# instance-based-loc/instance-based-loc

Hardware: AMD Instinct MI355X
Metric: query-frames localized/sec (embed+match+register) (higher is better)
Workload: dtype f16 (ViT MFMA operands, f32 accumulate) / f32+f64 (match, registration); 1 GPU; T: dinov2_vitb14 crops 224^2 (Q=7), 10000-instance memory (E=4), FPFH+RANSAC+coloured ICP on 5000-pt clouds, whole-memory evaluate; synthetic objects of extent U[0.15, 0.6] m on a 2.50 m grid (SURVEY 8d's U[0.2, 1.5] m re-scoped: its 5 000 points are too sparse to survive the radius-outlier removal); memory_instances=10000, points_per_object=5000, resident_feature_bytes_per_point=264, parallelism=frames-dp1+memory-replicated

## Files before the change

instance-based-loc_amd/csrc/vit.hip:

```cpp
#include "vit_kernels.h"

__global__ void ibl_set_prefix_kernel(float* __restrict__ x, const float* __restrict__ cls_pos, const float* __restrict__ reg, int B, int T,
                                      int n_prefix, int dim) {
    const int64_t i = (int64_t)blockIdx.x * blockDim.x + threadIdx.x;
    if (i >= (int64_t)B * n_prefix * dim) return;
    const int c = (int)(i % dim);
    const int64_t br = i / dim;
    const int b = (int)(br / n_prefix), r = (int)(br % n_prefix);
    x[((int64_t)b * T + r) * dim + c] = r == 0 ? cls_pos[c] : reg[(int64_t)(r - 1) * dim + c];
}

static int64_t vit_layout(const ibl_vit_desc* d, int batch, int64_t offs[IBL_VIT_WS_COUNT], int64_t* payload = nullptr) {
    const int64_t R = rows_pad((int64_t)batch * d->n_tokens);
    const int at = (d->flags & IBL_VIT_ACT_TERMS3) ? 3 : ((d->flags & IBL_VIT_ACT_TERMS2) ? 2 : 1);
    int64_t bytes[IBL_VIT_WS_COUNT];
    bytes[IBL_VIT_WS_X] = R * d->dim * 4;
    bytes[IBL_VIT_WS_XN] = R * d->dim * 2 * 3;
    bytes[IBL_VIT_WS_QKV] = R * 3 * d->dim * 2;
    bytes[IBL_VIT_WS_ATT] = R * d->dim * 2 * at;
    bytes[IBL_VIT_WS_HID] = R * d->mlp_dim * 2 * at;
    bytes[IBL_VIT_WS_FIN] = rows_pad(batch) * d->dim * 2;
    int64_t p = 0, sum = 0;
    for (int i = 0; i < IBL_VIT_WS_COUNT; ++i) {
        p = (p + 255) & ~(int64_t)255;
        offs[i] = p;
        p += bytes[i];
        sum += bytes[i];
    }
    if (payload) *payload = sum;
    return p;
}

extern "C" int64_t ibl_vit_workspace_bytes(const ibl_vit_desc* d, int batch) {
    if (!d || batch <= 0) return -1;
    int64_t offs[IBL_VIT_WS_COUNT], sum = 0;
    vit_layout(d, batch, offs, &sum);
    return sum + rows_pad(batch) * d->dim * 4 + 9 * 256;
}

extern "C" int ibl_vit_workspace_layout(const ibl_vit_desc* d, int batch, int64_t* offsets, int n) {
    if (!d || batch <= 0 || !offsets || n < 0 || n > IBL_VIT_WS_COUNT)
        return ibl_set_error(IBL_ERR_ARG, "ibl_vit_workspace_layout: bad argument");
    int64_t offs[IBL_VIT_WS_COUNT];
    vit_layout(d, batch, offs);
    for (int i = 0; i < n; ++i) offsets[i] = offs[i];
    return IBL_OK;
}

struct VitCtx {
    const ibl_vit_desc* d;
    const ibl_vit_weights* w;
    int batch;
    hipStream_t s;
    float* x;
    u16 *xn, *qkv, *att, *hid, *fin;
    int64_t Rn;
    int at;
    int n_prefix;
};


static int embed(const VitCtx& c, const void* patches) {
    const ibl_vit_desc* d = c.d;
    const ibl_vit_weights* w = c.w;
    const int D = d->dim, T = d->n_tokens, P = T - c.n_prefix;
    int st;
    GemmEpi e{};
    e.bias = w->b_patch; e.pos = w->pos_patch; e.out = c.x; e.ldo = D; e.tokens_per_crop = T; e.patches_per_crop = P;
    e.patch_row0 = c.n_prefix;
    st = gemm_launch(IBL_LINEAR_PATCH_F32, IBL_ACT_GELU_ERF, reinterpret_cast<const u16*>(patches), d->patch_k_pad,
                     reinterpret_cast<const u16*>(w->w_patch), d->patch_k_pad, c.batch * P, D, d->patch_k_pad, e, c.s);
    if (st) return st;
    if (w->w_patch_lo) {
        GemmEpi e2 = e;
        e2.bias = nullptr; e2.accumulate = 1; e2.alpha = 1.0f / IBL_VIT_SPLIT_SCALE; e2.algo_k = -1;
        st = gemm_launch(IBL_LINEAR_PATCH_F32, IBL_ACT_GELU_ERF, reinterpret_cast<const u16*>(patches), d->patch_k_pad,
                         reinterpret_cast<const u16*>(w->w_patch_lo), d->patch_k_pad, c.batch * P, D, d->patch_k_pad, e2, c.s);
        if (st) return st;
    }
    if (!(d->flags & IBL_VIT_NO_CLS)) {
        const int64_t n = (int64_t)c.batch * c.n_prefix * D;
        hipLaunchKernelGGL(ibl_set_prefix_kernel, dim3((unsigned)((n + 255) / 256)), dim3(256), 0, c.s, c.x, w->cls_pos, w->reg_tokens, c.batch,
                           T, c.n_prefix, D);
        IBL_LAUNCH_CHECK();
    }
    if (d->flags & IBL_VIT_PRE_LN) {
        st = launch_layernorm(c.x, D, c.Rn, D, w->ln_pre_g, w->ln_pre_b, d->ln_eps, c.x, D, 0, c.s);
        if (st) return st;
    }
    return IBL_OK;
}

static int resid_gemm(const VitCtx& c, bool cls_only, const u16* a, int64_t lda, int rows, int terms, int K, const void* w, const void* w_x,
                      const void* w_lo, const float* bias, const float* ls, const float* ls_lo) {
    const int D = c.d->dim;
    GemmEpi e{};
    e.bias = bias; e.scale = ls; e.out = c.x; e.ldo = cls_only ? (int64_t)c.d->n_tokens * D : D; e.alpha = 1.0f; e.algo_k = K;
    const int64_t kx = (int64_t)terms * K;
    int st = gemm_launch((ls || !gemm_resid_pre()) ? IBL_LINEAR_RESID_F32 : IBL_LINEAR_RESID_PRE_F32, IBL_ACT_GELU_ERF, a, lda,
                         reinterpret_cast<const u16*>(terms > 1 ? w_x : w), kx, rows, D, (int)kx, e, c.s);
    if (st) return st;
    if (!cls_only && terms == 1 && w_lo) {
        e.bias = nullptr; e.scale = ls_lo; e.algo_k = -1; e.alpha = 1.0f / IBL_VIT_SPLIT_SCALE;
        st = gemm_launch(ls_lo ? IBL_LINEAR_RESID_F32 : IBL_LINEAR_RESID_PRE_F32, IBL_ACT_GELU_ERF, a, K, reinterpret_cast<const u16*>(w_lo), K, rows,
                         D, K, e, c.s);
    }
    return st;
}

static int attention_half(const VitCtx& c, int l, const BlockTerms& t) {
    const ibl_vit_desc* d = c.d;
    const ibl_vit_layer* L = &c.w->layers[l];
    const int D = d->dim, T = d->n_tokens, H = d->heads;
    const int64_t TD = (int64_t)T * D;
    int st = launch_layernorm(c.x, D, c.Rn, D, L->ln1_g, L->ln1_b, d->ln_eps, c.xn, (int64_t)t.qkv * D, t.qkv, c.s);
    if (st) return st;
    if (!t.cls_only) {
        GemmEpi e{};
        e.bias = L->b_qkv; e.out = c.qkv; e.ldo = 3 * D; e.algo_k = D;
        st = gemm_launch(IBL_LINEAR_F16, IBL_ACT_GELU_ERF, c.xn, (int64_t)t.qkv * D, reinterpret_cast<const u16*>(t.qkv > 1 ? L->w_qkv_x : L->w_qkv),
                         (int64_t)t.qkv * D, (int)c.Rn, 3 * D, t.qkv * D, e, c.s);
        if (st) return st;
    } else {
        GemmEpi e{};
        e.bias = L->b_qkv + D; e.out = c.qkv + D; e.ldo = 3 * D;
        st = gemm_launch(IBL_LINEAR_F16, IBL_ACT_GELU_ERF, c.xn, D, reinterpret_cast<const u16*>(L->w_qkv) + (int64_t)D * D, D, (int)c.Rn, 2 * D, D, e,
                         c.s);
        if (st) return st;
        GemmEpi q{};
        q.bias = L->b_qkv; q.out = c.qkv; q.ldo = 3 * TD;
        st = gemm_launch(IBL_LINEAR_F16, IBL_ACT_GELU_ERF, c.xn, TD, reinterpret_cast<const u16*>(L->w_qkv), D, c.batch, D, D, q, c.s);
        if (st) return st;
    }
    if (c.w->rope_table) {
        st = run_rope(c.qkv, c.w->rope_table, c.batch, T, c.n_prefix, D, H, t.cls_only ? 1 : 0, c.s);
        if (st) return st;
    }
    st = run_attention(c.qkv, c.att, c.batch, T, D, H, t.cls_only ? 1 : 0, c.s, t.o);
    if (st) return st;
    return resid_gemm(c, t.cls_only, c.att, t.cls_only ? TD : (int64_t)t.o * D, t.cls_only ? c.batch : (int)c.Rn, t.o, D, L->w_o, L->w_o_x, L->w_o_lo,
                      L->b_o, L->ls1, L->ls1_lo);
}

static int mlp_half(const VitCtx& c, int l, const BlockTerms& t) {
    const ibl_vit_desc* d = c.d;
    const ibl_vit_layer* L = &c.w->layers[l];
    const int D = d->dim;
    int st = t.cls_only ? launch_layernorm(c.x, (int64_t)d->n_tokens * D, c.batch, D, L->ln2_g, L->ln2_b, d->ln_eps, c.fin, D, 1, c.s)
                        : launch_layernorm(c.x, D, c.Rn, D, L->ln2_g, L->ln2_b, d->ln_eps, c.xn, (int64_t)t.fc1 * D, t.fc1, c.s);
    if (st) return st;
    const u16* mlp_in = t.cls_only ? c.fin : c.xn;
    const int mlp_rows = t.cls_only ? c.batch : (int)c.Rn;
    GemmEpi e{};
    e.bias = L->b_fc1; e.out = c.hid; e.ldo = (int64_t)t.fc2 * d->mlp_dim; e.algo_k = D;
    const int epi = t.fc2 == 3 ? IBL_LINEAR_GELU_F16_X3 : (t.fc2 == 2 ? IBL_LINEAR_GELU_F16_X2 : IBL_LINEAR_GELU_F16);
    const int act = (d->flags & IBL_VIT_QUICK_GELU) ? IBL_ACT_QUICK_GELU : ((d->flags & IBL_VIT_TANH_GELU) ? IBL_ACT_GELU_TANH : IBL_ACT_GELU_ERF);
    st = gemm_launch(epi, act, mlp_in, (int64_t)t.fc1 * D, reinterpret_cast<const u16*>(t.fc1 > 1 ? L->w_fc1_x : L->w_fc1), (int64_t)t.fc1 * D, mlp_rows,
                     d->mlp_dim, t.fc1 * D, e, c.s);
    if (st) return st;
    return resid_gemm(c, t.cls_only, c.hid, (int64_t)t.fc2 * d->mlp_dim, mlp_rows, t.fc2, d->mlp_dim, L->w_fc2, L->w_fc2_x, L->w_fc2_lo, L->b_fc2,
                      L->ls2, L->ls2_lo);
}

static int head(const VitCtx& c, float* out) {
    const ibl_vit_desc* d = c.d;
    const ibl_vit_weights* w = c.w;
    const int D = d->dim, T = d->n_tokens;
    int st;
    if (d->flags & IBL_VIT_OUT_ALL_TOKENS) {
        if (d->flags & IBL_VIT_FINAL_LN) {
            st = launch_layernorm(c.x, D, c.Rn, D, w->ln_f_g, w->ln_f_b, d->ln_eps, out, D, 0, c.s);
            if (st) return st;
        } else {
            IBL_HIP_CHECK(hipMemcpyAsync(out, c.x, c.Rn * D * 4, hipMemcpyDeviceToDevice, c.s));
        }
        return IBL_OK;
    }
    if (d->flags & IBL_VIT_PROJ) {
        if (!(d->flags & IBL_VIT_FINAL_LN)) return ibl_set_error(IBL_ERR_UNSUPPORTED, "projection needs final LN");
        GemmEpi e{};
        e.bias = nullptr; e.out = out; e.ldo = d->out_dim;
        if (w->w_proj_x) {
            st = launch_layernorm(c.x, (int64_t)T * D, c.batch, D, w->ln_f_g, w->ln_f_b, d->ln_eps, c.xn, (int64_t)3 * D, 3, c.s);
            if (st) return st;
            e.algo_k = D;
            return gemm_launch(IBL_LINEAR_F32, IBL_ACT_GELU_ERF, c.xn, (int64_t)3 * D, reinterpret_cast<const u16*>(w->w_proj_x), (int64_t)3 * D, c.batch,
                               d->out_dim, 3 * D, e, c.s);
        }
        st = launch_layernorm(c.x, (int64_t)T * D, c.batch, D, w->ln_f_g, w->ln_f_b, d->ln_eps, c.fin, D, 1, c.s);
        if (st) return st;
        return gemm_launch(IBL_LINEAR_F32, IBL_ACT_GELU_ERF, c.fin, D, reinterpret_cast<const u16*>(w->w_proj), D, c.batch, d->out_dim, D, e, c.s);
    }
    if (d->flags & IBL_VIT_FINAL_LN) {
        st = launch_layernorm(c.x, (int64_t)T * D, c.batch, D, w->ln_f_g, w->ln_f_b, d->ln_eps, out, D, 0, c.s);
        if (st) return st;
    } else {
        IBL_HIP_CHECK(hipMemcpy2DAsync(out, (size_t)D * 4, c.x, (size_t)T * D * 4, (size_t)D * 4, c.batch,
                                       hipMemcpyDeviceToDevice, c.s));
    }
    return IBL_OK;
}

extern "C" int ibl_vit_forward(const ibl_vit_desc* d, const ibl_vit_weights* w, const void* patches, int batch,
                               float* out, void* workspace, int64_t workspace_bytes, void* stream) {
    if (!d || !w || !patches || !out || !workspace) return ibl_set_error(IBL_ERR_ARG, "ibl_vit_forward: null pointer");
    if (batch <= 0) return ibl_set_error(IBL_ERR_ARG, "ibl_vit_forward: batch must be positive");
    const bool no_cls = (d->flags & IBL_VIT_NO_CLS) != 0;
    const int D = d->dim, T = d->n_tokens, H = d->heads;
    const int n_reg = d->n_registers, n_prefix = no_cls ? 0 : 1 + n_reg, P = T - n_prefix;
    if (n_reg < 0 || (no_cls && n_reg != 0))
        return ibl_set_error(IBL_ERR_ARG, "ibl_vit_forward: n_registers %d%s", n_reg, no_cls ? " with IBL_VIT_NO_CLS: registers follow a class token" : " is negative");
    if (P < 1) return ibl_set_error(IBL_ERR_ARG, "ibl_vit_forward: n_tokens %d leaves no patch row after a prefix of %d", T, n_prefix);
    if (n_reg > 0 && !w->reg_tokens) return ibl_set_error(IBL_ERR_ARG, "ibl_vit_forward: n_registers %d without reg_tokens", n_reg);
    if (w->rope_table && (reinterpret_cast<uintptr_t>(w->rope_table) & 15))
        return ibl_set_error(IBL_ERR_ARG, "ibl_vit_forward: rope_table must be 16-byte aligned");
    if (no_cls && !(d->flags & IBL_VIT_OUT_ALL_TOKENS))
        return ibl_set_error(IBL_ERR_UNSUPPORTED, "ibl_vit_forward: IBL_VIT_NO_CLS needs IBL_VIT_OUT_ALL_TOKENS: without a class token there is no row to return");
    if ((d->flags & IBL_VIT_QUICK_GELU) && (d->flags & IBL_VIT_TANH_GELU))
        return ibl_set_error(IBL_ERR_ARG, "ibl_vit_forward: IBL_VIT_QUICK_GELU and IBL_VIT_TANH_GELU are both set");
    if (no_cls && T < 1) return ibl_set_error(IBL_ERR_ARG, "ibl_vit_forward: n_tokens %d with IBL_VIT_NO_CLS", T);
    if (D != H * 64) return ibl_set_error(IBL_ERR_UNSUPPORTED, "ibl_vit_forward: head_dim must be 64");
    if (D % 128 || d->mlp_dim % 128 || d->patch_k_pad % 64 || D > 1024)
        return ibl_set_error(IBL_ERR_UNSUPPORTED, "ibl_vit_forward: dim/mlp_dim %% 128, patch_k_pad %% 64, dim <= 1024");
    if (d->n_blocks_run < 0 || d->n_blocks_run > d->depth || d->depth > IBL_VIT_MAX_LAYERS)
        return ibl_set_error(IBL_ERR_ARG, "ibl_vit_forward: bad depth");
    if (workspace_bytes < ibl_vit_workspace_bytes(d, batch))
        return ibl_set_error(IBL_ERR_ARG, "ibl_vit_forward: workspace too small");

    int64_t offs[IBL_VIT_WS_COUNT];
    const int64_t end = vit_layout(d, batch, offs);
    unsigned char* base = reinterpret_cast<unsigned char*>((reinterpret_cast<uintptr_t>(workspace) + 255) & ~(uintptr_t)255);
    if ((base - reinterpret_cast<unsigned char*>(workspace)) + end > workspace_bytes)
        return ibl_set_error(IBL_ERR_ARG, "ibl_vit_forward: workspace too small");
    auto ws16 = [&](int i) { return reinterpret_cast<u16*>(base + offs[i]); };
    const VitCtx c{d, w, batch, (hipStream_t)stream, reinterpret_cast<float*>(base + offs[IBL_VIT_WS_X]), ws16(IBL_VIT_WS_XN), ws16(IBL_VIT_WS_QKV),
                   ws16(IBL_VIT_WS_ATT), ws16(IBL_VIT_WS_HID), ws16(IBL_VIT_WS_FIN), (int64_t)batch * T,
                   (d->flags & IBL_VIT_ACT_TERMS3) ? 3 : ((d->flags & IBL_VIT_ACT_TERMS2) ? 2 : 1), n_prefix};
    BlockTerms terms[IBL_VIT_MAX_LAYERS];
    int st;
    for (int l = 0; l < d->n_blocks_run; ++l) {
        terms[l] = block_terms(d, w, l);
        if ((st = check_block_terms("ibl_vit_forward", l, terms[l], c.at)) != IBL_OK) return st;
    }
    if ((st = embed(c, patches)) != IBL_OK) return st;
    for (int l = 0; l < d->n_blocks_run; ++l) {
        if ((st = attention_half(c, l, terms[l])) != IBL_OK) return st;
        if ((st = mlp_half(c, l, terms[l])) != IBL_OK) return st;
    }
    return head(c, out);
}
```

instance-based-loc_amd/csrc/vit_gemm.hip:

```cpp
#include <atomic>

#include "vit_kernels.h"

enum { EPI_BIAS_H16 = 0, EPI_BIAS_GELU_H16 = 1, EPI_RESID_F32 = 2, EPI_PATCH_F32 = 3, EPI_BIAS_F32 = 4,
       EPI_RESID_PRE_F32 = 5,
       EPI_BIAS_GELU_H16KX2 = 6, EPI_BIAS_GELU_H16KX3 = 7 };

constexpr int GBK = 64;

__device__ __forceinline__ int key_act(int r) { return r & 7; }
__device__ __forceinline__ int key_w(int r) { return (((r >> 4) & 3) << 1) | ((r >> 1) & 1); }
__device__ __forceinline__ int key_pair(int r) { return (((r >> 3) & 3) << 1) | ((r >> 1) & 1); }

typedef float f32x2 __attribute__((ext_vector_type(2)));
__device__ __forceinline__ f32x2 gelu_erf2(f32x2 v) {
    f32x2 z;
    z.x = fabsf(v.x) * 0.70710678118654752f;
    z.y = fabsf(v.y) * 0.70710678118654752f;
    const f32x2 d = z * 0.3275911f + 1.0f;
    f32x2 t;
    t.x = __builtin_amdgcn_rcpf(d.x);
    t.y = __builtin_amdgcn_rcpf(d.y);
    f32x2 p = t * 1.061405429f + -1.453152027f;
    p = p * t + 1.421413741f;
    p = p * t + -0.284496736f;
    p = p * t + 0.254829592f;
    const f32x2 a = (z * -1.4426950408889634f) * z;
    f32x2 e;
    e.x = __builtin_amdgcn_exp2f(a.x);
    e.y = __builtin_amdgcn_exp2f(a.y);
    const f32x2 u = 1.0f - (p * t) * e;
    return (z * u) * 0.70710678118654752f + v * 0.5f;
}

__device__ __forceinline__ f32x2 quick_gelu2(f32x2 v) {
    const f32x2 a = v * -2.4554669595930157f;
    f32x2 e;
    e.x = __builtin_amdgcn_exp2f(a.x);
    e.y = __builtin_amdgcn_exp2f(a.y);
    const f32x2 d = e + 1.0f;
    f32x2 r;
    r.x = __builtin_amdgcn_rcpf(d.x);
    r.y = __builtin_amdgcn_rcpf(d.y);
    return v * r;
}

__device__ __forceinline__ f32x2 tanh_gelu2(f32x2 v) {
    const f32x2 u = v * v;
    const f32x2 k = u * 0.044715f + 1.0f;
    const f32x2 w = v * k;
    const f32x2 a = w * -2.3022081985131374f;
    f32x2 e;
    e.x = __builtin_amdgcn_exp2f(a.x);
    e.y = __builtin_amdgcn_exp2f(a.y);
    const f32x2 d = e + 1.0f;
    f32x2 r;
    r.x = __builtin_amdgcn_rcpf(d.x);
    r.y = __builtin_amdgcn_rcpf(d.y);
    return v * r;
}

#ifdef IBL_GEMM_STAMPS
__device__ long long ibl_gemm_stamps[512 * 16 * 4];
__device__ int ibl_gemm_stamp_iter[512];
#define GEMM_STAMP(k)                                                                                  \
    do {                                                                                               \
        if (threadIdx.x == 0 && blockIdx.x < 512 && stamp_it < 16)                                     \
            ibl_gemm_stamps[(blockIdx.x * 16 + stamp_it) * 4 + (k)] = (long long)__builtin_amdgcn_s_memtime(); \
    } while (0)
extern "C" int ibl_gemm_stamps_read(long long* dst, int n) {
    return hipMemcpyFromSymbol(dst, HIP_SYMBOL(ibl_gemm_stamps), sizeof(long long) * n) == hipSuccess ? 0 : -1;
}
extern "C" int ibl_gemm_stamps_clear() {
    static long long zeros[512 * 16 * 4];
    return hipMemcpyToSymbol(HIP_SYMBOL(ibl_gemm_stamps), zeros, sizeof(zeros)) == hipSuccess ? 0 : -1;
}
#else
#define GEMM_STAMP(k)
#endif

template <int EPI, int ACT, bool T256>
__global__ __launch_bounds__(T256 ? 512 : 256, T256 ? 1 : 2) void ibl_gemm_f16_tn(const u16* __restrict__ A, int64_t lda, const u16* __restrict__ W,
                                                                                int64_t ldw, int M, int N, int K, GemmEpi epi) {
#if defined(__HIP_DEVICE_COMPILE__)
    constexpr int MI = T256 ? 8 : 4, WM = 2, WN = T256 ? 4 : 2, BK = GBK, NS = 2;
    constexpr bool PIPE = T256;
    constexpr int BM = WM * MI * 16, BN = WN * 64, NW = WM * WN;
    constexpr int LDS_ROW = BK * 2;
    constexpr int CPR = BK / 8, RPI = 64 / CPR;
    constexpr int A_BYTES = BM * LDS_ROW, W_BYTES = BN * LDS_ROW, STAGE = A_BYTES + W_BYTES;
    constexpr int GA = BM / RPI / NW, GW = BN / RPI / NW;
    extern __shared__ __attribute__((aligned(16))) unsigned char smem[];

    const int tid = threadIdx.x;
    const int lane = tid & 63, wave = tid >> 6;
    const int wm = wave / WN, wn = wave % WN;
    constexpr bool NAT = EPI == EPI_RESID_F32 || EPI == EPI_RESID_PRE_F32;
    constexpr bool PRE = EPI == EPI_RESID_PRE_F32;
    constexpr bool QGELU = ACT == IBL_ACT_QUICK_GELU, TGELU = ACT == IBL_ACT_GELU_TANH;
    constexpr int GT = EPI == EPI_BIAS_GELU_H16KX3 ? 3 : (EPI == EPI_BIAS_GELU_H16KX2 ? 2 : 1);
    constexpr bool GELU = EPI == EPI_BIAS_GELU_H16 || GT > 1;
    static_assert(GELU || ACT == IBL_ACT_GELU_ERF, "an activation with an epilogue that applies none");
    constexpr bool PAIR = EPI == EPI_BIAS_H16 || GELU;
    constexpr int PAIR_STORES = GT * 2 * MI;
#define KEYW(r) (NAT ? key_act(r) : (PAIR ? key_pair(r) : key_w(r)))
    const int nbn = N / BN;
    const int nbm = (M + BM - 1) / BM;
    const int nwg = nbn * nbm;
    __amdgpu_buffer_rsrc_t a_rsrc, w_rsrc;
    unsigned a_off[GA], w_off[GW];
    int row0, col0;
#define GEMM_SET_TILE(t)                                                                           \
    do {                                                                                           \
        int _bid = (t);                                                                            \
        {                                                                                          \
            const int _q = nwg / 8, _r = nwg % 8, _xcd = _bid % 8;                                 \
            _bid = (_xcd < _r ? _xcd * (_q + 1) : _r * (_q + 1) + (_xcd - _r) * _q) + _bid / 8;    \
        }                                                                                          \
        row0 = (_bid / nbn) * BM;                                                                  \
        col0 = (_bid % nbn) * BN;                                                                  \
        a_rsrc = __builtin_amdgcn_make_buffer_rsrc((void*)(A + (int64_t)row0 * lda), 0, -1, 0x00020000); \
        w_rsrc = __builtin_amdgcn_make_buffer_rsrc((void*)(W + (int64_t)col0 * ldw), 0, -1, 0x00020000); \
        _Pragma("unroll") for (int _i = 0; _i < GA; ++_i) {                                        \
            const int _rr = (wave + NW * _i) * RPI + lane / CPR, _pch = lane % CPR;                \
            int _ar = _rr;                                                                         \
            if (row0 + _ar >= M) _ar = M - 1 - row0;                                               \
            a_off[_i] = (unsigned)(((int64_t)_ar * lda + ((_pch ^ key_act(_rr)) << 3)) * 2);  \
        }                                                                                          \
        _Pragma("unroll") for (int _i = 0; _i < GW; ++_i) {                                        \
            const int _rr = (wave + NW * _i) * RPI + lane / CPR, _pch = lane % CPR;                \
            w_off[_i] = (unsigned)(((int64_t)_rr * ldw + ((_pch ^ KEYW(_rr)) << 3)) * 2);          \
        }                                                                                          \
    } while (0)
    int tile = blockIdx.x;
    GEMM_SET_TILE(tile);
#define GEMM_GLDS(buf, kt)                                                                                              \
    do {                                                                                                                \
        const int64_t _ko = (int64_t)(kt) * BK;                                                                         \
        _Pragma("unroll") for (int _i = 0; _i < GA; ++_i)                                                               \
            __builtin_amdgcn_raw_ptr_buffer_load_lds(a_rsrc, (__attribute__((address_space(3))) void*)(smem + (buf) * STAGE + (wave + NW * _i) * 1024), \
                                                     16, a_off[_i], (unsigned)(_ko * 2), 0, 0);                          \
        _Pragma("unroll") for (int _i = 0; _i < GW; ++_i)                                                               \
            __builtin_amdgcn_raw_ptr_buffer_load_lds(w_rsrc, (__attribute__((address_space(3))) void*)(smem + (buf) * STAGE + A_BYTES + (wave + NW * _i) * 1024), \
                                                     16, w_off[_i], (unsigned)(_ko * 2), 0, 0);                          \
    } while (0)

    f32x4 acc[MI][4];
    const int nk = K / BK;
    constexpr int NP = GA + GW;
    const int fr = lane & 15, fg = lane >> 4;
    int arow[MI], wrow[4];
#pragma unroll
    for (int i = 0; i < MI; ++i) arow[i] = wm * (MI * 16) + i * 16 + fr;
#pragma unroll
    for (int j = 0; j < 4; ++j)
        wrow[j] = NAT ? wn * 64 + 16 * j + fr
                      : (PAIR ? wn * 64 + 32 * (j >> 1) + 8 * (fr >> 2) + 4 * (j & 1) + (fr & 3) : wn * 64 + 16 * (fr >> 2) + 4 * j + (fr & 3));
#define GEMM_PIECE(stage, pc)                                                                                                       \
    do {                                                                                                                            \
        const int64_t _ko = (int64_t)(stage) * BK;                                                                                  \
        unsigned char* _dst = smem + ((stage) & 1) * STAGE;                                                                         \
        if ((pc) < GA)                                                                                                              \
            __builtin_amdgcn_raw_ptr_buffer_load_lds(a_rsrc, (__attribute__((address_space(3))) void*)(_dst + (wave + NW * (pc)) * 1024), 16,   \
                                                     a_off[(pc) < GA ? (pc) : 0], (unsigned)(_ko * 2), 0, 0);                               \
        else                                                                                                                        \
            __builtin_amdgcn_raw_ptr_buffer_load_lds(w_rsrc, (__attribute__((address_space(3))) void*)(_dst + A_BYTES + (wave + NW * ((pc) - GA)) * 1024), \
                                                     16, w_off[(pc) >= GA ? (pc) - GA : 0], (unsigned)(_ko * 2), 0, 0);                     \
    } while (0)
#define FRAG_W(buf, ks, j) (*reinterpret_cast<const h16x8*>(smem + (buf) * STAGE + A_BYTES + wrow[j] * LDS_ROW + (((4 * (ks) + fg) ^ KEYW(wrow[j])) << 4)))
#define FRAG_A(buf, ks, i) (*reinterpret_cast<const h16x8*>(smem + (buf) * STAGE + arow[i] * LDS_ROW + (((4 * (ks) + fg) ^ key_act(arow[i])) << 4)))
    static_assert(MI % 2 == 0, "pipelined loop: groups in halves");
    constexpr int HA = MI / 4, N2B = MI - HA;
    constexpr int NL = MI + 4;
    constexpr int LB = (NL + MI - 2) / (MI - 1);
    constexpr int LA = (NL + N2B - 2) / (N2B - 1);
    constexpr int NSLOT = N2B + MI;
    static_assert(!PIPE || NP <= 2 * NSLOT, "pieces per stage exceed the slots of a step");
    bool first_tile = true;
    bool stores_pending = false;
#ifdef IBL_GEMM_STAMPS
    int stamp_it = 0;
#endif
    for (;;) {
    GEMM_STAMP(0);
    if constexpr (PRE) {
        const int nbp = col0 + wn * 64 + 4 * fg;
        const float ia = 1.0f / epi.alpha;
        if (row0 + BM <= M) {
            const float* const xb = reinterpret_cast<const float*>(epi.out) + (int64_t)(row0 + wm * (MI * 16) + fr) * epi.ldo + nbp;
            const int64_t gstride = 16 * epi.ldo;
#pragma unroll
            for (int i = 0; i < MI; ++i)
#pragma unroll
                for (int j = 0; j < 4; ++j) {
                    const float4 x4 = *reinterpret_cast<const float4*>(xb + i * gstride + 16 * j);
                    acc[i][j] = f32x4{x4.x, x4.y, x4.z, x4.w};
                }
        } else {
#pragma unroll
            for (int i = 0; i < MI; ++i) {
                int row = row0 + wm * (MI * 16) + i * 16 + fr;
                row = row < M ? row : M - 1;
                const float* xr = reinterpret_cast<const float*>(epi.out) + (int64_t)row * epi.ldo + nbp;
#pragma unroll
                for (int j = 0; j < 4; ++j) {
                    const float4 x4 = *reinterpret_cast<const float4*>(xr + 16 * j);
                    acc[i][j] = f32x4{x4.x, x4.y, x4.z, x4.w};
                }
            }
        }
        if (epi.bias) {
#pragma unroll
            for (int j = 0; j < 4; ++j) {
                const float4 b4 = *reinterpret_cast<const float4*>(epi.bias + nbp + 16 * j);
#pragma unroll
                for (int i = 0; i < MI; ++i) {
                    acc[i][j][0] += b4.x; acc[i][j][1] += b4.y; acc[i][j][2] += b4.z; acc[i][j][3] += b4.w;
                }
            }
        }
        if (epi.alpha != 1.0f) {
#pragma unroll
            for (int i = 0; i < MI; ++i)
#pragma unroll
                for (int j = 0; j < 4; ++j) acc[i][j] *= ia;
        }
#pragma unroll
        for (int i = 0; i < MI; ++i)
            asm volatile("" : "+v"(acc[i][0]), "+v"(acc[i][1]), "+v"(acc[i][2]), "+v"(acc[i][3]));
    } else {
#pragma unroll
    for (int i = 0; i < MI; ++i)
#pragma unroll
        for (int j = 0; j < 4; ++j) acc[i][j] = f32x4{0.f, 0.f, 0.f, 0.f};
    }
    if constexpr (PIPE) {
#define GEMM_SLOT(u, stage)                                                                        \
    do {                                                                                           \
        if ((u) < NP) GEMM_PIECE(stage, (u) < NP ? (u) : 0);                                       \
        if (NSLOT + (u) < NP) GEMM_PIECE(stage, NSLOT + (u) < NP ? NSLOT + (u) : 0);               \
    } while (0)
#define GEMM_PROLOGUE()                                                                            \
    do {                                                                                           \
        _Pragma("unroll") for (int _pc = 0; _pc < NP; ++_pc) GEMM_PIECE(0, _pc);                   \
        if (nk > 1) {                                    \
            _Pragma("unroll") for (int _g = 0; _g < N2B; ++_g) GEMM_SLOT(_g, 1);                   \
        }                                                                                          \
    } while (0)
        if (first_tile) GEMM_PROLOGUE();
        if (PAIR && stores_pending) {
            asm volatile("s_waitcnt vmcnt(%0)" ::"i"(PAIR_STORES) : "memory");
            asm volatile("s_waitcnt lgkmcnt(0)" ::: "memory");
            __builtin_amdgcn_s_barrier();
        } else {
            asm volatile("s_waitcnt vmcnt(0)" ::: "memory");
            __syncthreads();
        }
        GEMM_STAMP(1);
        __builtin_amdgcn_sched_barrier(0);
        h16x8 afA[MI], wfA[4], afB[MI], wfB[4];
#pragma unroll
        for (int j = 0; j < 4; ++j) wfA[j] = FRAG_W(0, 0, j);
#pragma unroll
        for (int i = 0; i < MI; ++i) afA[i] = FRAG_A(0, 0, i);
        for (int kt = 0; kt < nk; ++kt) {
            const int buf = kt & 1;
            const bool more1 = kt + 1 < nk, more2 = kt + 2 < nk;
#pragma unroll
            for (int g = 0; g < MI; ++g) {
#pragma unroll
                for (int j = 0; j < 4; ++j) acc[g][j] = IBL_MFMA(wfA[j], afA[g], acc[g][j], 0, 0, 0);
                __builtin_amdgcn_sched_barrier(0);
#pragma unroll
                for (int t = g * LB; t < (g + 1) * LB && t < NL; ++t) {
                    if (t < 8 && (t & 1) == 0) wfB[t / 2] = FRAG_W(buf, 1, t / 2);
                    else afB[t < 8 ? t / 2 : t - 4] = FRAG_A(buf, 1, t < 8 ? t / 2 : t - 4);
                }
                if (more1) GEMM_SLOT(N2B + g, kt + 1);
                __builtin_amdgcn_sched_barrier(0);
            }
#pragma unroll
            for (int g = 0; g < HA; ++g) {
#pragma unroll
                for (int j = 0; j < 4; ++j) acc[g][j] = IBL_MFMA(wfB[j], afB[g], acc[g][j], 0, 0, 0);
            }
            __builtin_amdgcn_sched_barrier(0);
            asm volatile("s_waitcnt vmcnt(0) lgkmcnt(0)" ::: "memory");
            __syncthreads();
            const int nb = buf ^ 1;
#pragma unroll
            for (int g = 0; g < N2B; ++g) {
                if (more1) {
#pragma unroll
                    for (int t = g * LA; t < (g + 1) * LA && t < NL; ++t) {
                        if (t < 8 && (t & 1) == 0) wfA[t / 2] = FRAG_W(nb, 0, t / 2);
                        else afA[t < 8 ? t / 2 : t - 4] = FRAG_A(nb, 0, t < 8 ? t / 2 : t - 4);
                    }
                }
#pragma unroll
                for (int j = 0; j < 4; ++j) acc[HA + g][j] = IBL_MFMA(wfB[j], afB[HA + g], acc[HA + g][j], 0, 0, 0);
                if (more2) GEMM_SLOT(g, kt + 2);
                __builtin_amdgcn_sched_barrier(0);
            }
        }
    } else {
    static_assert(NS == 2, "the vmcnt(0) that closes a step leaves no later stage in flight");
#pragma unroll
    for (int st = 0; st < NS - 1; ++st)
        if (st < nk) GEMM_GLDS(st, st);
    asm volatile("s_waitcnt vmcnt(0)" ::: "memory");
    __syncthreads();
    GEMM_STAMP(1);
    constexpr int KS = BK / 32, NG = KS * MI;
    constexpr int NGI = NG / 2;
    for (int kt = 0; kt < nk; ++kt) {
        const int buf = kt % NS;
        const bool more = kt + NS - 1 < nk;
        const int64_t ko = (int64_t)(kt + NS - 1) * BK;
        unsigned char* nxt = smem + ((kt + NS - 1) % NS) * STAGE;
        const unsigned char* pa = smem + buf * STAGE;
        const unsigned char* pw = pa + A_BYTES;
#pragma unroll
        for (int ks = 0; ks < KS; ++ks) {
            const int ch = 4 * ks + fg;
            h16x8 af[MI], wf[4];
#pragma unroll
            for (int j = 0; j < 4; ++j) wf[j] = *reinterpret_cast<const h16x8*>(pw + wrow[j] * LDS_ROW + ((ch ^ KEYW(wrow[j])) << 4));
#pragma unroll
            for (int i = 0; i < MI; ++i) af[i] = *reinterpret_cast<const h16x8*>(pa + arow[i] * LDS_ROW + ((ch ^ key_act(arow[i])) << 4));
#pragma unroll
            for (int i = 0; i < MI; ++i) {
#pragma unroll
                for (int j = 0; j < 4; ++j)
                    acc[i][j] = IBL_MFMA(wf[j], af[i], acc[i][j], 0, 0, 0);
                const int g = ks * MI + i;
#pragma unroll
                for (int pc = (g < NGI ? g * NP / NGI : NP); pc < (g < NGI ? (g + 1) * NP / NGI : NP); ++pc) {
                    if (more) {
                        if (pc < GA)
                            __builtin_amdgcn_raw_ptr_buffer_load_lds(a_rsrc, (__attribute__((address_space(3))) void*)(nxt + (wave + NW * pc) * 1024), 16,
                                                                     a_off[pc], (unsigned)(ko * 2), 0, 0);
                        else
                            __builtin_amdgcn_raw_ptr_buffer_load_lds(w_rsrc, (__attribute__((address_space(3))) void*)(nxt + A_BYTES + (wave + NW * (pc - GA)) * 1024), 16,
                                                                     w_off[pc - GA], (unsigned)(ko * 2), 0, 0);
                    }
                }
            }
        }
        asm volatile("s_waitcnt vmcnt(0)" ::: "memory");
        __syncthreads();
    }
    }
    GEMM_STAMP(2);
    const int erow0 = row0, ecol0 = col0;
    float bb[2][8];
    if constexpr (PAIR) {
        const int nbp = ecol0 + wn * 64 + 8 * fg;
#pragma unroll
        for (int j2 = 0; j2 < 2; ++j2)
#pragma unroll
            for (int h = 0; h < 2; ++h) {
                const float4 b4 = epi.bias ? *reinterpret_cast<const float4*>(epi.bias + nbp + 32 * j2 + 4 * h) : make_float4(0.f, 0.f, 0.f, 0.f);
                bb[j2][4 * h] = b4.x; bb[j2][4 * h + 1] = b4.y; bb[j2][4 * h + 2] = b4.z; bb[j2][4 * h + 3] = b4.w;
            }
        asm volatile("" ::"v"(bb[0][0]), "v"(bb[0][1]), "v"(bb[0][2]), "v"(bb[0][3]), "v"(bb[0][4]), "v"(bb[0][5]), "v"(bb[0][6]), "v"(bb[0][7]),
                     "v"(bb[1][0]), "v"(bb[1][1]), "v"(bb[1][2]), "v"(bb[1][3]), "v"(bb[1][4]), "v"(bb[1][5]), "v"(bb[1][6]), "v"(bb[1][7]));
    }
    float4 b4[4], s4[4];
    if constexpr (NAT && !PRE) {
        const int nbq = ecol0 + wn * 64 + 4 * fg;
#pragma unroll
        for (int j = 0; j < 4; ++j) {
            b4[j] = epi.bias ? *reinterpret_cast<const float4*>(epi.bias + nbq + 16 * j) : make_float4(0.f, 0.f, 0.f, 0.f);
            s4[j] = epi.scale ? *reinterpret_cast<const float4*>(epi.scale + nbq + 16 * j) : make_float4(1.f, 1.f, 1.f, 1.f);
        }
#pragma unroll
        for (int j = 0; j < 4; ++j)
            asm volatile("" ::"v"(b4[j].x), "v"(b4[j].y), "v"(b4[j].z), "v"(b4[j].w), "v"(s4[j].x), "v"(s4[j].y), "v"(s4[j].z), "v"(s4[j].w));
    }
    tile += gridDim.x;
    const bool has_next = PIPE && tile < nwg;
    if constexpr (PIPE) {
        if (has_next) {
            GEMM_SET_TILE(tile);
            GEMM_PROLOGUE();
        }
    }


    if (PRE) {
        const int nb = ecol0 + wn * 64 + 4 * fg;
        const float al = epi.alpha;
        if (erow0 + BM <= M) {
            float* const obase = reinterpret_cast<float*>(epi.out) + (int64_t)(erow0 + wm * (MI * 16) + fr) * epi.ldo + nb;
            const int64_t gstride = 16 * epi.ldo;
#pragma unroll
            for (int i = 0; i < MI; ++i)
#pragma unroll
                for (int j = 0; j < 4; ++j)
                    *reinterpret_cast<float4*>(obase + i * gstride + 16 * j) =
                        make_float4(acc[i][j][0] * al, acc[i][j][1] * al, acc[i][j][2] * al, acc[i][j][3] * al);
        } else {
#pragma unroll
            for (int i = 0; i < MI; ++i) {
                const int row = erow0 + wm * (MI * 16) + i * 16 + fr;
                if (row >= M) continue;
                float* orow = reinterpret_cast<float*>(epi.out) + (int64_t)row * epi.ldo + nb;
#pragma unroll
                for (int j = 0; j < 4; ++j)
                    *reinterpret_cast<float4*>(orow + 16 * j) = make_float4(acc[i][j][0] * al, acc[i][j][1] * al, acc[i][j][2] * al, acc[i][j][3] * al);
            }
        }
    } else if (NAT) {
        const int nb = ecol0 + wn * 64 + 4 * fg;
#define RESID_RMW(X, I, PTR)                                                                                                        \
        _Pragma("unroll") for (int j = 0; j < 4; ++j) {                                                                             \
            float4 x = X[j];                                                                                                        \
            x.x += (acc[I][j][0] + b4[j].x) * s4[j].x; x.y += (acc[I][j][1] + b4[j].y) * s4[j].y;                                   \
            x.z += (acc[I][j][2] + b4[j].z) * s4[j].z; x.w += (acc[I][j][3] + b4[j].w) * s4[j].w;                                   \
            *reinterpret_cast<float4*>((PTR) + 16 * j) = x;                                                                         \
        }
        if (erow0 + BM <= M) {
            float* const obase = reinterpret_cast<float*>(epi.out) + (int64_t)(erow0 + wm * (MI * 16) + fr) * epi.ldo + nb;
            const int64_t gstride = 16 * epi.ldo;
            f32x4 xa[4], xb[4];
#define RMW_LOAD(X, PTR)                                                                                                            \
            do {                                                                                                                    \
                const float* _p = (PTR);                                                                                            \
                asm volatile("global_load_dwordx4 %0, %1, off" : "=&v"(X[0]) : "v"(_p) : "memory");                                 \
                asm volatile("global_load_dwordx4 %0, %1, off offset:64" : "=&v"(X[1]) : "v"(_p) : "memory");                       \
                asm volatile("global_load_dwordx4 %0, %1, off offset:128" : "=&v"(X[2]) : "v"(_p) : "memory");                      \
                asm volatile("global_load_dwordx4 %0, %1, off offset:192" : "=&v"(X[3]) : "v"(_p) : "memory");                      \
            } while (0)
#define RMW_WAIT(N, X) asm volatile("s_waitcnt vmcnt(" #N ")" : "+v"(X[0]), "+v"(X[1]), "+v"(X[2]), "+v"(X[3])::"memory")
#define RMW_STORE(X, I, PTR)                                                                                                        \
            do {                                                                                                                    \
                float* _p = (PTR);                                                                                                  \
                f32x4 _v[4];                                                                                                        \
                _Pragma("unroll") for (int j = 0; j < 4; ++j) {                                                                     \
                    _v[j][0] = X[j][0] + (acc[I][j][0] + b4[j].x) * s4[j].x; _v[j][1] = X[j][1] + (acc[I][j][1] + b4[j].y) * s4[j].y; \
                    _v[j][2] = X[j][2] + (acc[I][j][2] + b4[j].z) * s4[j].z; _v[j][3] = X[j][3] + (acc[I][j][3] + b4[j].w) * s4[j].w; \
                }                                                                                                                   \
                asm volatile("global_store_dwordx4 %0, %1, off" ::"v"(_p), "v"(_v[0]) : "memory");                                  \
                asm volatile("global_store_dwordx4 %0, %1, off offset:64" ::"v"(_p), "v"(_v[1]) : "memory");                        \
                asm volatile("global_store_dwordx4 %0, %1, off offset:128" ::"v"(_p), "v"(_v[2]) : "memory");                       \
                asm volatile("global_store_dwordx4 %0, %1, off offset:192" ::"v"(_p), "v"(_v[3]) : "memory");                       \
            } while (0)
            static_assert(MI % 2 == 0, "read-modify-write epilogue: row groups in pairs");
            RMW_LOAD(xa, obase);
#pragma unroll
            for (int i = 0; i < MI; i += 2) {
                RMW_LOAD(xb, obase + (i + 1) * gstride);
                if (i == 0) RMW_WAIT(4, xa); else RMW_WAIT(8, xa);
                RMW_STORE(xa, i, obase + i * gstride);
                if (i + 2 < MI) {
                    RMW_LOAD(xa, obase + (i + 2) * gstride);
                    RMW_WAIT(8, xb);
                } else {
                    RMW_WAIT(4, xb);
                }
                RMW_STORE(xb, i + 1, obase + (i + 1) * gstride);
            }
#undef RMW_LOAD
#undef RMW_WAIT
#undef RMW_STORE
        } else {
#pragma unroll
            for (int i = 0; i < MI; ++i) {
                const int row = erow0 + wm * (MI * 16) + i * 16 + fr;
                if (row >= M) continue;
                float* orow = reinterpret_cast<float*>(epi.out) + (int64_t)row * epi.ldo + nb;
                float4 xr[4];
#pragma unroll
                for (int j = 0; j < 4; ++j) xr[j] = *reinterpret_cast<const float4*>(orow + 16 * j);
                RESID_RMW(xr, i, orow)
            }
        }
#undef RESID_RMW
    } else if (PAIR) {
        const int nb = ecol0 + wn * 64 + 8 * fg;
#define PAIR_STORE(I, OROW)                                                                                                         \
        _Pragma("unroll") for (int j2 = 0; j2 < 2; ++j2) {                                                                          \
            float v[8];                                                                                                             \
            _Pragma("unroll") for (int t = 0; t < 8; t += 2) {                                                                      \
                f32x2 x = {acc[I][2 * j2 + (t >> 2)][t & 3], acc[I][2 * j2 + (t >> 2)][(t & 3) + 1]};                               \
                x += f32x2{bb[j2][t], bb[j2][t + 1]};                                                                               \
                if (GELU) x = QGELU ? quick_gelu2(x) : (TGELU ? tanh_gelu2(x) : gelu_erf2(x));                                      \
                v[t] = x.x; v[t + 1] = x.y;                                                                                         \
            }                                                                                                                       \
            const uint4 hi4 = make_uint4(f2h_pk(v[0], v[1]), f2h_pk(v[2], v[3]), f2h_pk(v[4], v[5]), f2h_pk(v[6], v[7]));           \
            *reinterpret_cast<uint4*>((OROW) + 32 * j2) = hi4;                                                                      \
            if (GT > 1) {                                                                                                           \
                const unsigned hw_[4] = {hi4.x, hi4.y, hi4.z, hi4.w};                                                               \
                unsigned lw_[4], sw_[4];                                                                                            \
                _Pragma("unroll") for (int t = 0; t < 4; ++t) {                                                                     \
                    const float h0 = h2f((u16)(hw_[t] & 0xFFFFu)), h1 = h2f((u16)(hw_[t] >> 16));                                   \
                    sw_[t] = f2h_pk(h0 * (1.0f / IBL_VIT_SPLIT_SCALE), h1 * (1.0f / IBL_VIT_SPLIT_SCALE));                          \
                    lw_[t] = f2h_pk((v[2 * t] - h0) * IBL_VIT_SPLIT_SCALE, (v[2 * t + 1] - h1) * IBL_VIT_SPLIT_SCALE);              \
                }                                                                                                                   \
                if (GT == 3) *reinterpret_cast<uint4*>((OROW) + N + 32 * j2) = make_uint4(lw_[0], lw_[1], lw_[2], lw_[3]);          \
                *reinterpret_cast<uint4*>((OROW) + (GT - 1) * (int64_t)N + 32 * j2) = make_uint4(sw_[0], sw_[1], sw_[2], sw_[3]);   \
            }                                                                                                                       \
        }
        if (erow0 + BM <= M) {
            u16* const obase = reinterpret_cast<u16*>(epi.out) + (int64_t)(erow0 + wm * (MI * 16) + fr) * epi.ldo + nb;
            const int64_t gstride = 16 * epi.ldo;
#pragma unroll
            for (int i = 0; i < MI; ++i) { PAIR_STORE(i, obase + i * gstride) }
            stores_pending = true;
        } else {
            stores_pending = false;
#pragma unroll
            for (int i = 0; i < MI; ++i) {
                const int row = erow0 + wm * (MI * 16) + i * 16 + fr;
                if (row >= M) continue;
                u16* orow = reinterpret_cast<u16*>(epi.out) + (int64_t)row * epi.ldo + nb;
                PAIR_STORE(i, orow)
            }
        }
#undef PAIR_STORE
    } else {
    const int n0 = ecol0 + wn * 64 + 16 * fg;
    float bias[16];
#pragma unroll
    for (int q = 0; q < 4; ++q) {
        float4 b4 = make_float4(0.f, 0.f, 0.f, 0.f);
        if (epi.bias) b4 = *reinterpret_cast<const float4*>(epi.bias + n0 + 4 * q);
        bias[4 * q] = b4.x; bias[4 * q + 1] = b4.y; bias[4 * q + 2] = b4.z; bias[4 * q + 3] = b4.w;
    }
#pragma unroll
    for (int i = 0; i < MI; ++i) {
        const int row = erow0 + wm * (MI * 16) + i * 16 + fr;
        if (row >= M) continue;
        float v[16];
#pragma unroll
        for (int j = 0; j < 4; ++j)
#pragma unroll
            for (int r = 0; r < 4; ++r) v[4 * j + r] = acc[i][j][r] + bias[4 * j + r];
        if (EPI == EPI_PATCH_F32) {
            const int b = row / epi.patches_per_crop, p = row - b * epi.patches_per_crop;
            const int64_t orow = (int64_t)b * epi.tokens_per_crop + epi.patch_row0 + p;
            float4* o = reinterpret_cast<float4*>(reinterpret_cast<float*>(epi.out) + orow * epi.ldo + n0);
            if (epi.accumulate) {
#pragma unroll
                for (int q = 0; q < 4; ++q) {
                    float4 xx = o[q];
                    xx.x = fmaf(v[4 * q], epi.alpha, xx.x); xx.y = fmaf(v[4 * q + 1], epi.alpha, xx.y);
                    xx.z = fmaf(v[4 * q + 2], epi.alpha, xx.z); xx.w = fmaf(v[4 * q + 3], epi.alpha, xx.w);
                    o[q] = xx;
                }
            } else {
                const float4* ps = reinterpret_cast<const float4*>(epi.pos + (int64_t)p * N + n0);
#pragma unroll
                for (int q = 0; q < 4; ++q) {
                    const float4 pp = ps[q];
                    o[q] = make_float4(v[4 * q] + pp.x, v[4 * q + 1] + pp.y, v[4 * q + 2] + pp.z, v[4 * q + 3] + pp.w);
                }
            }
        } else {
            float4* o = reinterpret_cast<float4*>(reinterpret_cast<float*>(epi.out) + (int64_t)row * epi.ldo + n0);
#pragma unroll
            for (int q = 0; q < 4; ++q) o[q] = make_float4(v[4 * q], v[4 * q + 1], v[4 * q + 2], v[4 * q + 3]);
        }
    }
    }
    GEMM_STAMP(3);
#ifdef IBL_GEMM_STAMPS
    ++stamp_it;
#endif
    if (!has_next) break;
    first_tile = false;
    }
#undef GEMM_PROLOGUE
#undef GEMM_SLOT
#undef GEMM_PIECE
#undef FRAG_W
#undef FRAG_A
#undef GEMM_GLDS
#undef GEMM_SET_TILE
#endif
}

template <int EPI, int ACT, bool T256>
static int launch_gemm_cfg(const u16* A, int64_t lda, const u16* W, int64_t ldw, int M, int N, int K, const GemmEpi& epi, hipStream_t s) {
    constexpr int BM = T256 ? 256 : 128, BN = BM;
    const int nwg = (N / BN) * ((M + BM - 1) / BM);
    const size_t lds = 2 * (size_t)(BM + BN) * GBK * 2;
    static std::atomic<unsigned long long> attr_set{0};
    int dev = 0;
    IBL_HIP_CHECK(hipGetDevice(&dev));
    const unsigned long long bit = 1ull << (dev & 63);
    if (!(attr_set.load(std::memory_order_acquire) & bit)) {
        IBL_HIP_CHECK(hipFuncSetAttribute(reinterpret_cast<const void*>(&ibl_gemm_f16_tn<EPI, ACT, T256>),
                                          hipFuncAttributeMaxDynamicSharedMemorySize, (int)lds));
        attr_set.fetch_or(bit, std::memory_order_release);
    }
    int grid = nwg;
    if (T256) {
        static std::atomic<int> n_cu{0};
        int cus = n_cu.load(std::memory_order_relaxed);
        if (cus == 0) {
            IBL_HIP_CHECK(hipDeviceGetAttribute(&cus, hipDeviceAttributeMultiprocessorCount, dev));
            cus = cus >= 8 ? cus / 8 * 8 : 8;
            n_cu.store(cus, std::memory_order_relaxed);
        }
        if (grid > cus) grid = cus;
    }
    void* tok;
    ibl_prof_begin(IBL_PROF_GEMM, 2.0 * (double)M * (double)N * (double)(epi.algo_k < 0 ? 0 : (epi.algo_k ? epi.algo_k : K)), s, &tok);
    hipLaunchKernelGGL((ibl_gemm_f16_tn<EPI, ACT, T256>), dim3(grid), dim3(T256 ? 512 : 256), lds, s, A, lda, W, ldw, M, N, K, epi);
    ibl_prof_end(tok, s);
    IBL_LAUNCH_CHECK();
    return IBL_OK;
}

bool gemm_resid_pre() {
    static int v = -1;
    if (v < 0) { const char* e = getenv("IBL_GEMM_RESID_PRE"); v = (e && atoi(e)) ? 1 : 0; }
    return v == 1;
}

template <int EPI, int ACT>
static int launch_gemm(const u16* A, int64_t lda, const u16* W, int64_t ldw, int M, int N, int K, const GemmEpi& epi,
                       hipStream_t s) {
    if (M <= 0) return IBL_OK;
    if (N % 128 != 0 || K % GBK != 0)
        return ibl_set_error(IBL_ERR_ARG, "gemm: N (%d) must be a multiple of 128 and K (%d) of 64", N, K);
    if (N % 256 == 0 && M >= 4096) return launch_gemm_cfg<EPI, ACT, true>(A, lda, W, ldw, M, N, K, epi, s);
    return launch_gemm_cfg<EPI, ACT, false>(A, lda, W, ldw, M, N, K, epi, s);
}

int gemm_launch(int epi, int act, const u16* A, int64_t lda, const u16* W, int64_t ldw, int M, int N, int K, const GemmEpi& e, hipStream_t s) {
    if (epi < EPI_BIAS_H16 || epi > EPI_BIAS_GELU_H16KX3) return ibl_set_error(IBL_ERR_ARG, "%s: unknown epilogue %d", "gemm", epi);
    switch (act * 8 + epi) {
#define GEMM_ROW(EPI, ACT) \
    case (ACT) * 8 + (EPI): return launch_gemm<EPI, ACT>(A, lda, W, ldw, M, N, K, e, s)
        GEMM_ROW(EPI_BIAS_H16, IBL_ACT_GELU_ERF);
        GEMM_ROW(EPI_BIAS_GELU_H16, IBL_ACT_GELU_ERF);
        GEMM_ROW(EPI_RESID_F32, IBL_ACT_GELU_ERF);
        GEMM_ROW(EPI_PATCH_F32, IBL_ACT_GELU_ERF);
        GEMM_ROW(EPI_BIAS_F32, IBL_ACT_GELU_ERF);
        GEMM_ROW(EPI_RESID_PRE_F32, IBL_ACT_GELU_ERF);
        GEMM_ROW(EPI_BIAS_GELU_H16KX2, IBL_ACT_GELU_ERF);
        GEMM_ROW(EPI_BIAS_GELU_H16KX3, IBL_ACT_GELU_ERF);
        GEMM_ROW(EPI_BIAS_GELU_H16, IBL_ACT_QUICK_GELU);
        GEMM_ROW(EPI_BIAS_GELU_H16KX2, IBL_ACT_QUICK_GELU);
        GEMM_ROW(EPI_BIAS_GELU_H16KX3, IBL_ACT_QUICK_GELU);
        GEMM_ROW(EPI_BIAS_GELU_H16, IBL_ACT_GELU_TANH);
        GEMM_ROW(EPI_BIAS_GELU_H16KX2, IBL_ACT_GELU_TANH);
        GEMM_ROW(EPI_BIAS_GELU_H16KX3, IBL_ACT_GELU_TANH);
#undef GEMM_ROW
    }
    return ibl_set_error(IBL_ERR_ARG, "%s: activation %d with epilogue %d (0, or a known one with a GELU epilogue)", "gemm", act, epi);
}

static_assert(IBL_LINEAR_F16 == EPI_BIAS_H16 && IBL_LINEAR_GELU_F16 == EPI_BIAS_GELU_H16 && IBL_LINEAR_RESID_F32 == EPI_RESID_F32 &&
                  IBL_LINEAR_PATCH_F32 == EPI_PATCH_F32 && IBL_LINEAR_F32 == EPI_BIAS_F32 && IBL_LINEAR_RESID_PRE_F32 == EPI_RESID_PRE_F32 &&
                  IBL_LINEAR_GELU_F16_X2 == EPI_BIAS_GELU_H16KX2 && IBL_LINEAR_GELU_F16_X3 == EPI_BIAS_GELU_H16KX3,
              "the header's epilogue numbers are the kernel's");
static_assert(sizeof(ibl_linear_desc) == 112, "activation fills the tail padding of ibl_linear_desc: its size is part of the ABI");

static bool pow2_positive(float a) {
    int e;
    return a >= 1.17549435e-38f && a <= 3.0e38f && frexpf(a, &e) == 0.5f;
}

static int linear_f16_run(const ibl_linear_desc* d, int act, int act_max, void* stream, const char* fn);

extern "C" int ibl_linear_f16_ex(const ibl_linear_desc* d, void* stream) {
    if (!d) return ibl_set_error(IBL_ERR_ARG, "ibl_linear_f16_ex: null descriptor");
    if (d->rows == 0) return IBL_OK;
    return linear_f16_run(d, d->activation, IBL_ACT_QUICK_GELU, stream, "ibl_linear_f16_ex");
}

extern "C" int ibl_linear_f16_act(const ibl_linear_desc* d, int activation, void* stream) {
    if (!d) return ibl_set_error(IBL_ERR_ARG, "ibl_linear_f16_act: null descriptor");
    if (d->activation != 0)
        return ibl_set_error(IBL_ERR_ARG, "ibl_linear_f16_act: the descriptor's activation field (%d) must be 0: the activation is the argument", d->activation);
    if (activation < IBL_ACT_GELU_ERF || activation > IBL_ACT_GELU_TANH)
        return ibl_set_error(IBL_ERR_ARG, "ibl_linear_f16_act: unknown activation %d (0, 1 or 2)", activation);
    if (d->rows == 0) return IBL_OK;
    return linear_f16_run(d, activation, IBL_ACT_GELU_TANH, stream, "ibl_linear_f16_act");
}

static int linear_f16_run(const ibl_linear_desc* d, int act, int act_max, void* stream, const char* fn) {
    if (!d->x || !d->W || !d->out) return ibl_set_error(IBL_ERR_ARG, "%s: null operand", fn);
    if (d->rows < 0 || d->rows > 0x7fffffff) return ibl_set_error(IBL_ERR_ARG, "%s: rows out of range", fn);
    const int n_out = d->n_out, n_in = d->n_in, epi = d->epilogue;
    if (n_out <= 0 || n_in <= 0 || n_out % 128 != 0 || n_in % GBK != 0)
        return ibl_set_error(IBL_ERR_ARG, "%s: n_out (%d) must be a positive multiple of 128 and n_in (%d) of 64", fn, n_out, n_in);
    if (epi < EPI_BIAS_H16 || epi > EPI_BIAS_GELU_H16KX3) return ibl_set_error(IBL_ERR_ARG, "%s: unknown epilogue %d", fn, epi);
    const bool gelu = epi == EPI_BIAS_GELU_H16 || epi == EPI_BIAS_GELU_H16KX2 || epi == EPI_BIAS_GELU_H16KX3;
    if (act != IBL_ACT_GELU_ERF && !(gelu && act > 0 && act <= act_max))
        return ibl_set_error(IBL_ERR_ARG, "%s: activation %d with epilogue %d (0, or a known one with a GELU epilogue)", fn, act, epi);
    const int terms = epi == EPI_BIAS_GELU_H16KX3 ? 3 : (epi == EPI_BIAS_GELU_H16KX2 ? 2 : 1);
    if ((d->ldx & 7) || (d->ldw & 7) || (d->ldo & 7) || d->ldx < n_in || d->ldw < n_in || d->ldo < (int64_t)terms * n_out)
        return ibl_set_error(IBL_ERR_ARG, "%s: row strides must be >= the row length (%d in, %d out) and multiples of 8 elements", fn,
                             n_in, terms * n_out);
    GemmEpi e{};
    e.bias = d->bias;
    e.out = d->out;
    e.ldo = d->ldo;
    if (epi == EPI_RESID_F32) e.scale = d->scale;
    if (epi == EPI_RESID_PRE_F32 || (epi == EPI_PATCH_F32 && d->accumulate)) {
        if (!pow2_positive(d->alpha)) return ibl_set_error(IBL_ERR_ARG, "%s: alpha (%g) must be a positive power of two", fn, (double)d->alpha);
        e.alpha = d->alpha;
    }
    if (epi == EPI_PATCH_F32) {
        if (d->patches_per_crop <= 0 || d->tokens_per_crop <= d->patches_per_crop || d->rows % d->patches_per_crop != 0)
            return ibl_set_error(IBL_ERR_ARG, "%s: patch scatter needs 0 < patches_per_crop (%d) < tokens_per_crop (%d) and whole crops (%lld rows)", fn,
                                 d->patches_per_crop, d->tokens_per_crop, (long long)d->rows);
        if (d->accumulate != 0 && d->accumulate != 1) return ibl_set_error(IBL_ERR_ARG, "%s: accumulate must be 0 or 1", fn);
        if (!d->accumulate && !d->pos) return ibl_set_error(IBL_ERR_ARG, "%s: null position rows without accumulate", fn);
        e.pos = d->pos;
        e.tokens_per_crop = d->tokens_per_crop;
        e.patches_per_crop = d->patches_per_crop;
        e.patch_row0 = 1;
        e.accumulate = d->accumulate;
    }
    return gemm_launch(epi, act, reinterpret_cast<const u16*>(d->x), d->ldx, reinterpret_cast<const u16*>(d->W), d->ldw, (int)d->rows, n_out, n_in,
                       e, reinterpret_cast<hipStream_t>(stream));
}

extern "C" int ibl_linear_f16(const void* x, int64_t ldx, const void* W, int64_t ldw, const float* bias, const float* scale,
                               int64_t rows, int n_out, int n_in, int epilogue, void* out, int64_t ldo, void* stream) {
    if (epilogue != EPI_BIAS_H16 && epilogue != EPI_BIAS_GELU_H16 && epilogue != EPI_RESID_F32 && epilogue != EPI_BIAS_F32 && rows != 0)
        return ibl_set_error(IBL_ERR_ARG, "ibl_linear_f16: unknown epilogue %d", epilogue);
    ibl_linear_desc d{};
    d.x = x; d.ldx = ldx; d.W = W; d.ldw = ldw; d.bias = bias; d.scale = scale; d.out = out; d.ldo = ldo;
    d.rows = rows; d.n_out = n_out; d.n_in = n_in; d.epilogue = epilogue;
    d.alpha = 1.0f;
    if (epilogue == EPI_RESID_F32 && !scale && gemm_resid_pre()) d.epilogue = EPI_RESID_PRE_F32;
    return ibl_linear_f16_ex(&d, stream);
}
```

instance-based-loc_amd/csrc/vit_kernels.h:

```cpp
#pragma once
#include <hip/hip_runtime.h>
#include <hip/hip_fp16.h>

#include "ibl_common.h"
#include "ibloc.h"

typedef __attribute__((ext_vector_type(8))) _Float16 h16x8;
typedef __attribute__((ext_vector_type(4))) float f32x4;
typedef unsigned short u16;

__device__ __forceinline__ u16 f2h(float f) {
    const _Float16 h = (_Float16)__builtin_amdgcn_fmed3f(f, -65504.0f, 65504.0f);
    return __builtin_bit_cast(u16, h);
}

__device__ __forceinline__ float h2f(u16 h) { return (float)__builtin_bit_cast(_Float16, h); }

typedef _Float16 h16x2 __attribute__((ext_vector_type(2)));
__device__ __forceinline__ unsigned f2h_pk(float a, float b) {
    typedef float f32x2_ __attribute__((ext_vector_type(2)));
    h16x2 r = __builtin_convertvector(f32x2_{a, b}, h16x2);
    const h16x2 hi = {(_Float16)65504.0f, (_Float16)65504.0f};
    r = __builtin_elementwise_min(r, hi);
    r = __builtin_elementwise_max(r, -hi);
    return __builtin_bit_cast(unsigned, r);
}

struct GemmEpi {
    const float* bias;
    const float* scale;
    const float* pos;
    void* out;
    int64_t ldo;
    int tokens_per_crop;
    int patches_per_crop;
    int patch_row0;
    int accumulate;
    float alpha;
    int algo_k;
};

#define IBL_MFMA(a, b, c, x, y, z) __builtin_amdgcn_mfma_f32_16x16x32_f16(a, b, c, x, y, z)

static inline int64_t rows_pad(int64_t r) { return ibl_align_up(r, 128); }

#define VIT_INTERNAL __attribute__((visibility("hidden")))

VIT_INTERNAL int gemm_launch(int epi, int act, const u16* A, int64_t lda, const u16* W, int64_t ldw, int M, int N, int K, const GemmEpi& e,
                             hipStream_t s);
VIT_INTERNAL bool gemm_resid_pre();
VIT_INTERNAL int launch_layernorm(const float* x, int64_t ld_x, int64_t n_rows, int dim, const float* g, const float* b, float eps, void* out,
                                  int64_t ld_out, int terms, hipStream_t s);
VIT_INTERNAL int run_rope(u16* qkv, const float* table, int B, int T, int n_prefix, int D, int heads, int k_only, hipStream_t s);
VIT_INTERNAL int run_attention(const u16* qkv, u16* out, int B, int T, int D, int heads, int cls_only, hipStream_t s, int terms);
VIT_INTERNAL int ragged_offsets_check(const char* fn, const int32_t* seq_off, int batch, int* max_tokens);
VIT_INTERNAL int run_attention_ragged(const u16* qkv, u16* out, const int* seq_off, int B, int max_tokens, int D, int heads, int cls_only,
                                      hipStream_t s, int terms);

struct BlockTerms {
    bool cls_only;
    int qkv, o, fc1, fc2;
};

static inline BlockTerms block_terms(const ibl_vit_desc* d, const ibl_vit_weights* w, int l) {
    const ibl_vit_layer* L = &w->layers[l];
    BlockTerms t;
    t.cls_only = (l == d->n_blocks_run - 1) && !(d->flags & IBL_VIT_OUT_ALL_TOKENS);
    t.qkv = (!t.cls_only && L->w_qkv_x && L->qkv_terms > 1) ? L->qkv_terms : 1;
    t.o = (!t.cls_only && L->w_o_x && L->o_terms > 1) ? L->o_terms : 1;
    t.fc1 = (!t.cls_only && L->w_fc1_x && L->fc1_terms > 1) ? L->fc1_terms : 1;
    t.fc2 = (!t.cls_only && L->w_fc2_x && L->fc2_terms > 1) ? L->fc2_terms : 1;
    return t;
}

static inline int check_block_terms(const char* fn, int l, const BlockTerms& t, int at) {
    if (t.qkv > 3 || t.fc1 > 3) return ibl_set_error(IBL_ERR_ARG, "%s: layer %d: at most three operand terms", fn, l);
    if (t.o > at || t.fc2 > at || t.o > 3 || t.fc2 > 3)
        return ibl_set_error(IBL_ERR_ARG, "%s: layer %d: o_terms / fc2_terms %d / %d need IBL_VIT_ACT_TERMS%d in the descriptor", fn, l, t.o, t.fc2, t.o > t.fc2 ? t.o : t.fc2);
    return IBL_OK;
}
```

instance-based-loc_amd/csrc/vit_ragged.hip:

```cpp
#include "vit_kernels.h"

__global__ void ibl_set_prefix_ragged_kernel(float* __restrict__ x, const float* __restrict__ cls_pos, const float* __restrict__ reg,
                                             const int* __restrict__ seq_off, int B, int n_prefix, int dim) {
    const int64_t i = (int64_t)blockIdx.x * blockDim.x + threadIdx.x;
    if (i >= (int64_t)B * n_prefix * dim) return;
    const int c = (int)(i % dim);
    const int64_t br = i / dim;
    const int b = (int)(br / n_prefix), r = (int)(br % n_prefix);
    x[((int64_t)seq_off[b] + r) * dim + c] = r == 0 ? cls_pos[c] : reg[(int64_t)(r - 1) * dim + c];
}

__global__ void ibl_class_rows_kernel(uint4* __restrict__ rows, int64_t ld_rows, uint4* __restrict__ compact, int64_t ld_compact,
                                      const int* __restrict__ seq_off, int B, int n16, int scatter) {
    const int64_t i = (int64_t)blockIdx.x * blockDim.x + threadIdx.x;
    if (i >= (int64_t)B * n16) return;
    const int b = (int)(i / n16), c = (int)(i % n16);
    uint4* r = rows + (int64_t)seq_off[b] * ld_rows + c;
    uint4* k = compact + (int64_t)b * ld_compact + c;
    if (scatter) *r = *k;
    else *k = *r;
}

enum { RW_X = 0, RW_XN, RW_QKV, RW_ATT, RW_HID, RW_FIN, RW_CX, RW_CA, RW_COUNT };

static int act_terms(const ibl_vit_desc* d) { return (d->flags & IBL_VIT_ACT_TERMS3) ? 3 : ((d->flags & IBL_VIT_ACT_TERMS2) ? 2 : 1); }

static int64_t ragged_layout(const ibl_vit_desc* d, int64_t total_tokens, int batch, int64_t offs[RW_COUNT]) {
    const int64_t R = rows_pad(total_tokens), Bp = rows_pad(batch);
    const int at = act_terms(d);
    int64_t bytes[RW_COUNT];
    bytes[RW_X] = R * d->dim * 4;
    bytes[RW_XN] = R * d->dim * 2 * 3;
    bytes[RW_QKV] = R * 3 * d->dim * 2;
    bytes[RW_ATT] = R * d->dim * 2 * at;
    bytes[RW_HID] = R * d->mlp_dim * 2 * at;
    bytes[RW_FIN] = Bp * d->dim * 2;
    bytes[RW_CX] = Bp * d->dim * 4;
    bytes[RW_CA] = Bp * d->dim * 2;
    int64_t p = 0;
    for (int i = 0; i < RW_COUNT; ++i) {
        p = (p + 255) & ~(int64_t)255;
        offs[i] = p;
        p += bytes[i];
    }
    return p;
}

extern "C" int64_t ibl_vit_ragged_workspace_bytes(const ibl_vit_desc* d, int64_t total_tokens, int batch) {
    if (!d || batch <= 0 || total_tokens < batch || total_tokens > 0x7fffffff) return -1;
    int64_t offs[RW_COUNT];
    return ragged_layout(d, total_tokens, batch, offs) + 256;
}

struct RaggedCtx {
    const ibl_vit_desc* d;
    const ibl_vit_weights* w;
    int batch;
    hipStream_t s;
    const int* seq_off;
    int max_tokens;
    float *x, *cx;
    u16 *xn, *qkv, *att, *hid, *fin, *ca;
    int64_t Rn;
    int n_prefix;
};

static int class_rows(const RaggedCtx& c, void* rows, int64_t ld_rows_bytes, void* compact, int row_bytes, int scatter) {
    const int n16 = row_bytes / 16;
    const int64_t n = (int64_t)c.batch * n16;
    hipLaunchKernelGGL(ibl_class_rows_kernel, dim3((unsigned)((n + 255) / 256)), dim3(256), 0, c.s, reinterpret_cast<uint4*>(rows),
                       ld_rows_bytes / 16, reinterpret_cast<uint4*>(compact), (int64_t)n16, c.seq_off, c.batch, n16, scatter);
    IBL_LAUNCH_CHECK();
    return IBL_OK;
}

static int embed(const RaggedCtx& c, const void* patches, const float* pos_rows) {
    const ibl_vit_desc* d = c.d;
    const ibl_vit_weights* w = c.w;
    const int D = d->dim;
    GemmEpi e{};
    e.bias = w->b_patch; e.pos = pos_rows; e.out = c.x; e.ldo = D; e.tokens_per_crop = (int)c.Rn; e.patches_per_crop = (int)c.Rn; e.patch_row0 = 0;
    int st = gemm_launch(IBL_LINEAR_PATCH_F32, IBL_ACT_GELU_ERF, reinterpret_cast<const u16*>(patches), d->patch_k_pad,
                         reinterpret_cast<const u16*>(w->w_patch), d->patch_k_pad, (int)c.Rn, D, d->patch_k_pad, e, c.s);
    if (st) return st;
    if (w->w_patch_lo) {
        GemmEpi e2 = e;
        e2.bias = nullptr; e2.accumulate = 1; e2.alpha = 1.0f / IBL_VIT_SPLIT_SCALE; e2.algo_k = -1;
        st = gemm_launch(IBL_LINEAR_PATCH_F32, IBL_ACT_GELU_ERF, reinterpret_cast<const u16*>(patches), d->patch_k_pad,
                         reinterpret_cast<const u16*>(w->w_patch_lo), d->patch_k_pad, (int)c.Rn, D, d->patch_k_pad, e2, c.s);
        if (st) return st;
    }
    const int64_t n = (int64_t)c.batch * c.n_prefix * D;
    hipLaunchKernelGGL(ibl_set_prefix_ragged_kernel, dim3((unsigned)((n + 255) / 256)), dim3(256), 0, c.s, c.x, w->cls_pos, w->reg_tokens,
                       c.seq_off, c.batch, c.n_prefix, D);
    IBL_LAUNCH_CHECK();
    return IBL_OK;
}

static int resid_gemm(const RaggedCtx& c, bool cls_only, float* out, const u16* a, int64_t lda, int rows, int terms, int K, const void* w,
                      const void* w_x, const void* w_lo, const float* bias, const float* ls, const float* ls_lo) {
    const int D = c.d->dim;
    GemmEpi e{};
    e.bias = bias; e.scale = ls; e.out = out; e.ldo = D; e.alpha = 1.0f; e.algo_k = K;
    const int64_t kx = (int64_t)terms * K;
    int st = gemm_launch((ls || !gemm_resid_pre()) ? IBL_LINEAR_RESID_F32 : IBL_LINEAR_RESID_PRE_F32, IBL_ACT_GELU_ERF, a, lda,
                         reinterpret_cast<const u16*>(terms > 1 ? w_x : w), kx, rows, D, (int)kx, e, c.s);
    if (st) return st;
    if (!cls_only && terms == 1 && w_lo) {
        e.bias = nullptr; e.scale = ls_lo; e.algo_k = -1; e.alpha = 1.0f / IBL_VIT_SPLIT_SCALE;
        st = gemm_launch(ls_lo ? IBL_LINEAR_RESID_F32 : IBL_LINEAR_RESID_PRE_F32, IBL_ACT_GELU_ERF, a, K, reinterpret_cast<const u16*>(w_lo), K, rows,
                         D, K, e, c.s);
    }
    return st;
}

static int attention_half(const RaggedCtx& c, int l, const BlockTerms& t) {
    const ibl_vit_desc* d = c.d;
    const ibl_vit_layer* L = &c.w->layers[l];
    const int D = d->dim, H = d->heads;
    int st = launch_layernorm(c.x, D, c.Rn, D, L->ln1_g, L->ln1_b, d->ln_eps, c.xn, (int64_t)t.qkv * D, t.qkv, c.s);
    if (st) return st;
    if (!t.cls_only) {
        GemmEpi e{};
        e.bias = L->b_qkv; e.out = c.qkv; e.ldo = 3 * D; e.algo_k = D;
        st = gemm_launch(IBL_LINEAR_F16, IBL_ACT_GELU_ERF, c.xn, (int64_t)t.qkv * D, reinterpret_cast<const u16*>(t.qkv > 1 ? L->w_qkv_x : L->w_qkv),
                         (int64_t)t.qkv * D, (int)c.Rn, 3 * D, t.qkv * D, e, c.s);
        if (st) return st;
        st = run_attention_ragged(c.qkv, c.att, c.seq_off, c.batch, c.max_tokens, D, H, 0, c.s, t.o);
        if (st) return st;
        return resid_gemm(c, false, c.x, c.att, (int64_t)t.o * D, (int)c.Rn, t.o, D, L->w_o, L->w_o_x, L->w_o_lo, L->b_o, L->ls1, L->ls1_lo);
    }
    GemmEpi e{};
    e.bias = L->b_qkv + D; e.out = c.qkv + D; e.ldo = 3 * D;
    st = gemm_launch(IBL_LINEAR_F16, IBL_ACT_GELU_ERF, c.xn, D, reinterpret_cast<const u16*>(L->w_qkv) + (int64_t)D * D, D, (int)c.Rn, 2 * D, D, e, c.s);
    if (st) return st;
    if ((st = class_rows(c, c.xn, (int64_t)D * 2, c.fin, D * 2, 0)) != IBL_OK) return st;
    GemmEpi q{};
    q.bias = L->b_qkv; q.out = c.ca; q.ldo = D;
    st = gemm_launch(IBL_LINEAR_F16, IBL_ACT_GELU_ERF, c.fin, D, reinterpret_cast<const u16*>(L->w_qkv), D, c.batch, D, D, q, c.s);
    if (st) return st;
    if ((st = class_rows(c, c.qkv, (int64_t)3 * D * 2, c.ca, D * 2, 1)) != IBL_OK) return st;
    st = run_attention_ragged(c.qkv, c.att, c.seq_off, c.batch, c.max_tokens, D, H, 1, c.s, 1);
    if (st) return st;
    if ((st = class_rows(c, c.att, (int64_t)D * 2, c.ca, D * 2, 0)) != IBL_OK) return st;
    if ((st = class_rows(c, c.x, (int64_t)D * 4, c.cx, D * 4, 0)) != IBL_OK) return st;
    return resid_gemm(c, true, c.cx, c.ca, D, c.batch, 1, D, L->w_o, L->w_o_x, L->w_o_lo, L->b_o, L->ls1, L->ls1_lo);
}

static int mlp_half(const RaggedCtx& c, int l, const BlockTerms& t) {
    const ibl_vit_desc* d = c.d;
    const ibl_vit_layer* L = &c.w->layers[l];
    const int D = d->dim;
    int st = t.cls_only ? launch_layernorm(c.cx, D, c.batch, D, L->ln2_g, L->ln2_b, d->ln_eps, c.fin, D, 1, c.s)
                        : launch_layernorm(c.x, D, c.Rn, D, L->ln2_g, L->ln2_b, d->ln_eps, c.xn, (int64_t)t.fc1 * D, t.fc1, c.s);
    if (st) return st;
    const u16* mlp_in = t.cls_only ? c.fin : c.xn;
    const int mlp_rows = t.cls_only ? c.batch : (int)c.Rn;
    GemmEpi e{};
    e.bias = L->b_fc1; e.out = c.hid; e.ldo = (int64_t)t.fc2 * d->mlp_dim; e.algo_k = D;
    const int epi = t.fc2 == 3 ? IBL_LINEAR_GELU_F16_X3 : (t.fc2 == 2 ? IBL_LINEAR_GELU_F16_X2 : IBL_LINEAR_GELU_F16);
    const int act = (d->flags & IBL_VIT_QUICK_GELU) ? IBL_ACT_QUICK_GELU : ((d->flags & IBL_VIT_TANH_GELU) ? IBL_ACT_GELU_TANH : IBL_ACT_GELU_ERF);
    st = gemm_launch(epi, act, mlp_in, (int64_t)t.fc1 * D, reinterpret_cast<const u16*>(t.fc1 > 1 ? L->w_fc1_x : L->w_fc1), (int64_t)t.fc1 * D, mlp_rows,
                     d->mlp_dim, t.fc1 * D, e, c.s);
    if (st) return st;
    return resid_gemm(c, t.cls_only, t.cls_only ? c.cx : c.x, c.hid, (int64_t)t.fc2 * d->mlp_dim, mlp_rows, t.fc2, d->mlp_dim, L->w_fc2,
                      L->w_fc2_x, L->w_fc2_lo, L->b_fc2, L->ls2, L->ls2_lo);
}

static int head(const RaggedCtx& c, float* out, bool have_cx) {
    const ibl_vit_desc* d = c.d;
    const ibl_vit_weights* w = c.w;
    const int D = d->dim;
    int st;
    if (d->flags & IBL_VIT_OUT_ALL_TOKENS) {
        if (d->flags & IBL_VIT_FINAL_LN) return launch_layernorm(c.x, D, c.Rn, D, w->ln_f_g, w->ln_f_b, d->ln_eps, out, D, 0, c.s);
        IBL_HIP_CHECK(hipMemcpyAsync(out, c.x, c.Rn * D * 4, hipMemcpyDeviceToDevice, c.s));
        return IBL_OK;
    }
    if (!have_cx && (st = class_rows(c, c.x, (int64_t)D * 4, c.cx, D * 4, 0)) != IBL_OK) return st;
    if (d->flags & IBL_VIT_FINAL_LN) return launch_layernorm(c.cx, D, c.batch, D, w->ln_f_g, w->ln_f_b, d->ln_eps, out, D, 0, c.s);
    IBL_HIP_CHECK(hipMemcpyAsync(out, c.cx, (size_t)c.batch * D * 4, hipMemcpyDeviceToDevice, c.s));
    return IBL_OK;
}

extern "C" int ibl_vit_forward_ragged(const ibl_vit_desc* d, const ibl_vit_weights* w, const void* patches, const float* pos_rows,
                                      const int32_t* seq_off_dev, const int32_t* seq_off_host, int batch, float* out, void* workspace,
                                      int64_t workspace_bytes, void* stream) {
    const char* fn = "ibl_vit_forward_ragged";
    if (!d || !w || !patches || !pos_rows || !seq_off_dev || !seq_off_host || !out || !workspace)
        return ibl_set_error(IBL_ERR_ARG, "%s: null pointer", fn);
    if (batch <= 0) return ibl_set_error(IBL_ERR_ARG, "%s: batch must be positive", fn);
    if (w->rope_table) return ibl_set_error(IBL_ERR_UNSUPPORTED, "%s: a rotary table (DINOv3) is not supported: it would have to be ragged too", fn);
    if (d->flags & IBL_VIT_NO_CLS) return ibl_set_error(IBL_ERR_UNSUPPORTED, "%s: IBL_VIT_NO_CLS (SigLIP) is not supported: a class-token model is needed", fn);
    if (d->flags & (IBL_VIT_PROJ | IBL_VIT_PRE_LN))
        return ibl_set_error(IBL_ERR_UNSUPPORTED, "%s: IBL_VIT_PROJ / IBL_VIT_PRE_LN (CLIP) are not supported: its position table is not defined off its grid", fn);
    const int D = d->dim, H = d->heads, n_reg = d->n_registers, n_prefix = 1 + n_reg;
    if (n_reg < 0) return ibl_set_error(IBL_ERR_ARG, "%s: n_registers %d is negative", fn, n_reg);
    if (n_reg > 0 && !w->reg_tokens) return ibl_set_error(IBL_ERR_ARG, "%s: n_registers %d without reg_tokens", fn, n_reg);
    if ((d->flags & IBL_VIT_QUICK_GELU) && (d->flags & IBL_VIT_TANH_GELU))
        return ibl_set_error(IBL_ERR_ARG, "%s: IBL_VIT_QUICK_GELU and IBL_VIT_TANH_GELU are both set", fn);
    if (D != H * 64) return ibl_set_error(IBL_ERR_UNSUPPORTED, "%s: head_dim must be 64", fn);
    if (D % 128 || d->mlp_dim % 128 || d->patch_k_pad % 64 || D > 1024)
        return ibl_set_error(IBL_ERR_UNSUPPORTED, "%s: dim/mlp_dim %% 128, patch_k_pad %% 64, dim <= 1024", fn);
    if (d->n_blocks_run < 0 || d->n_blocks_run > d->depth || d->depth > IBL_VIT_MAX_LAYERS) return ibl_set_error(IBL_ERR_ARG, "%s: bad depth", fn);
    if ((reinterpret_cast<uintptr_t>(patches) & 15) || (reinterpret_cast<uintptr_t>(pos_rows) & 15) || (reinterpret_cast<uintptr_t>(seq_off_dev) & 3))
        return ibl_set_error(IBL_ERR_ARG, "%s: patches and pos_rows must be 16-byte, seq_off 4-byte aligned", fn);
    int st, max_tokens;
    if ((st = ragged_offsets_check(fn, seq_off_host, batch, &max_tokens)) != IBL_OK) return st;
    if (seq_off_host[0] != 0) return ibl_set_error(IBL_ERR_ARG, "%s: seq_off[0] must be 0", fn);
    for (int b = 0; b < batch; ++b)
        if (seq_off_host[b + 1] - seq_off_host[b] <= n_prefix)
            return ibl_set_error(IBL_ERR_ARG, "%s: crop %d has %d rows: no patch row after a prefix of %d", fn, b, seq_off_host[b + 1] - seq_off_host[b], n_prefix);
    const int64_t Rn = seq_off_host[batch];
    int64_t offs[RW_COUNT];
    const int64_t end = ragged_layout(d, Rn, batch, offs);
    unsigned char* base = reinterpret_cast<unsigned char*>((reinterpret_cast<uintptr_t>(workspace) + 255) & ~(uintptr_t)255);
    if ((base - reinterpret_cast<unsigned char*>(workspace)) + end > workspace_bytes) return ibl_set_error(IBL_ERR_ARG, "%s: workspace too small", fn);
    auto ws16 = [&](int i) { return reinterpret_cast<u16*>(base + offs[i]); };
    const RaggedCtx c{d, w, batch, (hipStream_t)stream, seq_off_dev, max_tokens, reinterpret_cast<float*>(base + offs[RW_X]),
                      reinterpret_cast<float*>(base + offs[RW_CX]), ws16(RW_XN), ws16(RW_QKV), ws16(RW_ATT), ws16(RW_HID), ws16(RW_FIN),
                      ws16(RW_CA), Rn, n_prefix};
    BlockTerms terms[IBL_VIT_MAX_LAYERS];
    const int at = act_terms(d);
    for (int l = 0; l < d->n_blocks_run; ++l) {
        terms[l] = block_terms(d, w, l);
        if ((st = check_block_terms(fn, l, terms[l], at)) != IBL_OK) return st;
    }
    if ((st = embed(c, patches, pos_rows)) != IBL_OK) return st;
    for (int l = 0; l < d->n_blocks_run; ++l) {
        if ((st = attention_half(c, l, terms[l])) != IBL_OK) return st;
        if ((st = mlp_half(c, l, terms[l])) != IBL_OK) return st;
    }
    return head(c, out, d->n_blocks_run > 0 && terms[d->n_blocks_run - 1].cls_only);
}
```

Before: 832.4 query-frames/s.

## Reuse the activation tile across split-weight terms in the two-term GEMM K loop

Adds a TERMS template parameter to the pipelined 256-tile f16 GEMM. For two-term (hi/lo split) rows it loads each activation K-block into LDS once and pairs it with both weight column halves. The second term is scaled by 1/64 in registers rather than reading a duplicated activation copy. This is meant to halve the activation traffic for the extended-K GEMMs, at the cost of extra per-fragment multiplies and a more intricate buffer schedule. Whether it runs depends on the model's term configuration.

```diff
diff --git a/instance-based-loc_amd/csrc/vit.hip b/instance-based-loc_amd/csrc/vit.hip
--- a/instance-based-loc_amd/csrc/vit.hip
+++ b/instance-based-loc_amd/csrc/vit.hip
@@ -98,7 +98,7 @@
     e.bias = bias; e.scale = ls; e.out = c.x; e.ldo = cls_only ? (int64_t)c.d->n_tokens * D : D; e.alpha = 1.0f; e.algo_k = K;
     const int64_t kx = (int64_t)terms * K;
     int st = gemm_launch((ls || !gemm_resid_pre()) ? IBL_LINEAR_RESID_F32 : IBL_LINEAR_RESID_PRE_F32, IBL_ACT_GELU_ERF, a, lda,
-                         reinterpret_cast<const u16*>(terms > 1 ? w_x : w), kx, rows, D, (int)kx, e, c.s);
+                         reinterpret_cast<const u16*>(terms > 1 ? w_x : w), kx, rows, D, (int)kx, e, c.s, terms);
     if (st) return st;
     if (!cls_only && terms == 1 && w_lo) {
         e.bias = nullptr; e.scale = ls_lo; e.algo_k = -1; e.alpha = 1.0f / IBL_VIT_SPLIT_SCALE;
@@ -119,7 +119,7 @@
         GemmEpi e{};
         e.bias = L->b_qkv; e.out = c.qkv; e.ldo = 3 * D; e.algo_k = D;
         st = gemm_launch(IBL_LINEAR_F16, IBL_ACT_GELU_ERF, c.xn, (int64_t)t.qkv * D, reinterpret_cast<const u16*>(t.qkv > 1 ? L->w_qkv_x : L->w_qkv),
-                         (int64_t)t.qkv * D, (int)c.Rn, 3 * D, t.qkv * D, e, c.s);
+                         (int64_t)t.qkv * D, (int)c.Rn, 3 * D, t.qkv * D, e, c.s, t.qkv);
         if (st) return st;
     } else {
         GemmEpi e{};
@@ -156,7 +156,7 @@
     const int epi = t.fc2 == 3 ? IBL_LINEAR_GELU_F16_X3 : (t.fc2 == 2 ? IBL_LINEAR_GELU_F16_X2 : IBL_LINEAR_GELU_F16);
     const int act = (d->flags & IBL_VIT_QUICK_GELU) ? IBL_ACT_QUICK_GELU : ((d->flags & IBL_VIT_TANH_GELU) ? IBL_ACT_GELU_TANH : IBL_ACT_GELU_ERF);
     st = gemm_launch(epi, act, mlp_in, (int64_t)t.fc1 * D, reinterpret_cast<const u16*>(t.fc1 > 1 ? L->w_fc1_x : L->w_fc1), (int64_t)t.fc1 * D, mlp_rows,
-                     d->mlp_dim, t.fc1 * D, e, c.s);
+                     d->mlp_dim, t.fc1 * D, e, c.s, t.fc1);
     if (st) return st;
     return resid_gemm(c, t.cls_only, c.hid, (int64_t)t.fc2 * d->mlp_dim, mlp_rows, t.fc2, d->mlp_dim, L->w_fc2, L->w_fc2_x, L->w_fc2_lo, L->b_fc2,
                       L->ls2, L->ls2_lo);
@@ -185,7 +185,7 @@
             if (st) return st;
             e.algo_k = D;
             return gemm_launch(IBL_LINEAR_F32, IBL_ACT_GELU_ERF, c.xn, (int64_t)3 * D, reinterpret_cast<const u16*>(w->w_proj_x), (int64_t)3 * D, c.batch,
-                               d->out_dim, 3 * D, e, c.s);
+                               d->out_dim, 3 * D, e, c.s, 3);
         }
         st = launch_layernorm(c.x, (int64_t)T * D, c.batch, D, w->ln_f_g, w->ln_f_b, d->ln_eps, c.fin, D, 1, c.s);
         if (st) return st;
diff --git a/instance-based-loc_amd/csrc/vit_gemm.hip b/instance-based-loc_amd/csrc/vit_gemm.hip
--- a/instance-based-loc_amd/csrc/vit_gemm.hip
+++ b/instance-based-loc_amd/csrc/vit_gemm.hip
@@ -79,10 +79,17 @@
 #define GEMM_STAMP(k)
 #endif
 
-template <int EPI, int ACT, bool T256>
+__host__ __device__ constexpr bool kx_new_a(int terms, int r) { return terms == 1 || r == 0; }
+__host__ __device__ constexpr int kx_col_w(int terms, int r) { return terms == 2 ? r : 0; }
+__host__ __device__ constexpr int kx_buf_a(int terms, int kb, int r) { return kb & 1; }
+__host__ __device__ constexpr int kx_buf_w(int terms, int kb, int r) { return terms == 2 ? r : (kb & 1); }
+__host__ __device__ constexpr bool kx_scale_a(int terms, int r) { return terms == 2 && r == 1; }
+
+template <int EPI, int ACT, bool T256, int TERMS>
 __global__ __launch_bounds__(T256 ? 512 : 256, T256 ? 1 : 2) void ibl_gemm_f16_tn(const u16* __restrict__ A, int64_t lda, const u16* __restrict__ W,
                                                                                 int64_t ldw, int M, int N, int K, GemmEpi epi) {
 #if defined(__HIP_DEVICE_COMPILE__)
+    static_assert(TERMS == 1 || (T256 && TERMS == 2), "the terms-aware K loop is the pipelined one, for two-term rows");
     constexpr int MI = T256 ? 8 : 4, WM = 2, WN = T256 ? 4 : 2, BK = GBK, NS = 2;
     constexpr bool PIPE = T256;
     constexpr int BM = WM * MI * 16, BN = WN * 64, NW = WM * WN;
@@ -93,7 +100,7 @@
     extern __shared__ __attribute__((aligned(16))) unsigned char smem[];
 
     const int tid = threadIdx.x;
-    const int lane = tid & 63, wave = tid >> 6;
+    const int lane = tid & 63, wave = TERMS > 1 ? __builtin_amdgcn_readfirstlane(tid >> 6) : tid >> 6;
     const int wm = wave / WN, wn = wave % WN;
     constexpr bool NAT = EPI == EPI_RESID_F32 || EPI == EPI_RESID_PRE_F32;
     constexpr bool PRE = EPI == EPI_RESID_PRE_F32;
@@ -147,6 +154,7 @@
 
     f32x4 acc[MI][4];
     const int nk = K / BK;
+    const int Kb = K / TERMS;
     constexpr int NP = GA + GW;
     const int fr = lane & 15, fg = lane >> 4;
     int arow[MI], wrow[4];
@@ -156,16 +164,17 @@
     for (int j = 0; j < 4; ++j)
         wrow[j] = NAT ? wn * 64 + 16 * j + fr
                       : (PAIR ? wn * 64 + 32 * (j >> 1) + 8 * (fr >> 2) + 4 * (j & 1) + (fr & 3) : wn * 64 + 16 * (fr >> 2) + 4 * j + (fr & 3));
-#define GEMM_PIECE(stage, pc)                                                                                                       \
+#define GEMM_PIECE(kb, r, pc)                                                                                                       \
     do {                                                                                                                            \
-        const int64_t _ko = (int64_t)(stage) * BK;                                                                                  \
-        unsigned char* _dst = smem + ((stage) & 1) * STAGE;                                                                         \
-        if ((pc) < GA)                                                                                                              \
-            __builtin_amdgcn_raw_ptr_buffer_load_lds(a_rsrc, (__attribute__((address_space(3))) void*)(_dst + (wave + NW * (pc)) * 1024), 16,   \
-                                                     a_off[(pc) < GA ? (pc) : 0], (unsigned)(_ko * 2), 0, 0);                               \
-        else                                                                                                                        \
-            __builtin_amdgcn_raw_ptr_buffer_load_lds(w_rsrc, (__attribute__((address_space(3))) void*)(_dst + A_BYTES + (wave + NW * ((pc) - GA)) * 1024), \
-                                                     16, w_off[(pc) >= GA ? (pc) - GA : 0], (unsigned)(_ko * 2), 0, 0);                     \
+        const int64_t _ko = (int64_t)(kb) * BK;                                                                                     \
+        if ((pc) < GA) {                                                                                                            \
+            if (kx_new_a(TERMS, r))                                                                                                 \
+                __builtin_amdgcn_raw_ptr_buffer_load_lds(a_rsrc, (__attribute__((address_space(3))) void*)(smem + kx_buf_a(TERMS, kb, r) * STAGE + (wave + NW * (pc)) * 1024), 16, \
+                                                         a_off[(pc) < GA ? (pc) : 0], (unsigned)(_ko * 2), 0, 0);                          \
+        } else {                                                                                                                    \
+            __builtin_amdgcn_raw_ptr_buffer_load_lds(w_rsrc, (__attribute__((address_space(3))) void*)(smem + kx_buf_w(TERMS, kb, r) * STAGE + A_BYTES + (wave + NW * ((pc) - GA)) * 1024), \
+                                                         16, w_off[(pc) >= GA ? (pc) - GA : 0], (unsigned)((_ko + kx_col_w(TERMS, r) * (int64_t)Kb) * 2), 0, 0); \
+        }                                                                                                                           \
     } while (0)
 #define FRAG_W(buf, ks, j) (*reinterpret_cast<const h16x8*>(smem + (buf) * STAGE + A_BYTES + wrow[j] * LDS_ROW + (((4 * (ks) + fg) ^ KEYW(wrow[j])) << 4)))
 #define FRAG_A(buf, ks, i) (*reinterpret_cast<const h16x8*>(smem + (buf) * STAGE + arow[i] * LDS_ROW + (((4 * (ks) + fg) ^ key_act(arow[i])) << 4)))
@@ -235,16 +244,16 @@
         for (int j = 0; j < 4; ++j) acc[i][j] = f32x4{0.f, 0.f, 0.f, 0.f};
     }
     if constexpr (PIPE) {
-#define GEMM_SLOT(u, stage)                                                                        \
+#define GEMM_SLOT(u, kb, r)                                                                        \
     do {                                                                                           \
-        if ((u) < NP) GEMM_PIECE(stage, (u) < NP ? (u) : 0);                                       \
-        if (NSLOT + (u) < NP) GEMM_PIECE(stage, NSLOT + (u) < NP ? NSLOT + (u) : 0);               \
+        if ((u) < NP) GEMM_PIECE(kb, r, (u) < NP ? (u) : 0);                                       \
+        if (NSLOT + (u) < NP) GEMM_PIECE(kb, r, NSLOT + (u) < NP ? NSLOT + (u) : 0);               \
     } while (0)
 #define GEMM_PROLOGUE()                                                                            \
     do {                                                                                           \
-        _Pragma("unroll") for (int _pc = 0; _pc < NP; ++_pc) GEMM_PIECE(0, _pc);                   \
+        _Pragma("unroll") for (int _pc = 0; _pc < NP; ++_pc) GEMM_PIECE(0, 0, _pc);                \
         if (nk > 1) {                                    \
-            _Pragma("unroll") for (int _g = 0; _g < N2B; ++_g) GEMM_SLOT(_g, 1);                   \
+            _Pragma("unroll") for (int _g = 0; _g < N2B; ++_g) GEMM_SLOT(_g, TERMS == 1 ? 1 : 0, TERMS == 1 ? 0 : 1);    \
         }                                                                                          \
     } while (0)
         if (first_tile) GEMM_PROLOGUE();
@@ -263,45 +272,60 @@
         for (int j = 0; j < 4; ++j) wfA[j] = FRAG_W(0, 0, j);
 #pragma unroll
         for (int i = 0; i < MI; ++i) afA[i] = FRAG_A(0, 0, i);
+        static_assert(IBL_VIT_SPLIT_SCALE == 64.0f, "0x2400 is 1 / 64");
+        constexpr unsigned RS_PK = 0x24002400u, ONE_PK = 0x3C003C00u;
+        constexpr bool SA = TERMS > 1;
+        int kb = 0, r = 0;
         for (int kt = 0; kt < nk; ++kt) {
-            const int buf = kt & 1;
+            const int r1 = TERMS == 1 || r + 1 == TERMS ? 0 : r + 1, kb1 = TERMS == 1 ? kt + 1 : (r + 1 == TERMS ? kb + 1 : kb);
+            const int r2 = TERMS == 1 || r1 + 1 == TERMS ? 0 : r1 + 1, kb2 = TERMS == 1 ? kt + 2 : (r1 + 1 == TERMS ? kb1 + 1 : kb1);
+            const int ab = TERMS == 1 ? kt & 1 : kx_buf_a(TERMS, kb, r), wb = TERMS == 1 ? kt & 1 : kx_buf_w(TERMS, kb, r);
+            const h16x2 fa2 = __builtin_bit_cast(h16x2, kx_scale_a(TERMS, r) ? RS_PK : ONE_PK);
+            const h16x8 fa = {fa2.x, fa2.y, fa2.x, fa2.y, fa2.x, fa2.y, fa2.x, fa2.y};
             const bool more1 = kt + 1 < nk, more2 = kt + 2 < nk;
+            if (SA) afA[0] *= fa;
 #pragma unroll
             for (int g = 0; g < MI; ++g) {
 #pragma unroll
                 for (int j = 0; j < 4; ++j) acc[g][j] = IBL_MFMA(wfA[j], afA[g], acc[g][j], 0, 0, 0);
+                if (SA && g + 1 < MI) afA[g + 1] *= fa;
                 __builtin_amdgcn_sched_barrier(0);
 #pragma unroll
                 for (int t = g * LB; t < (g + 1) * LB && t < NL; ++t) {
-                    if (t < 8 && (t & 1) == 0) wfB[t / 2] = FRAG_W(buf, 1, t / 2);
-                    else afB[t < 8 ? t / 2 : t - 4] = FRAG_A(buf, 1, t < 8 ? t / 2 : t - 4);
-                }
-                if (more1) GEMM_SLOT(N2B + g, kt + 1);
+                    if (t < 8 && (t & 1) == 0) wfB[t / 2] = FRAG_W(wb, 1, t / 2);
+                    else afB[t < 8 ? t / 2 : t - 4] = FRAG_A(ab, 1, t < 8 ? t / 2 : t - 4);
+                }
+                if (more1) GEMM_SLOT(N2B + g, kb1, r1);
                 __builtin_amdgcn_sched_barrier(0);
             }
+            if (SA) afB[0] *= fa;
 #pragma unroll
             for (int g = 0; g < HA; ++g) {
 #pragma unroll
                 for (int j = 0; j < 4; ++j) acc[g][j] = IBL_MFMA(wfB[j], afB[g], acc[g][j], 0, 0, 0);
+                if (SA) afB[g + 1] *= fa;
             }
             __builtin_amdgcn_sched_barrier(0);
             asm volatile("s_waitcnt vmcnt(0) lgkmcnt(0)" ::: "memory");
             __syncthreads();
-            const int nb = buf ^ 1;
+            const int nab = TERMS == 1 ? ab ^ 1 : kx_buf_a(TERMS, kb1, r1), nwb = TERMS == 1 ? wb ^ 1 : kx_buf_w(TERMS, kb1, r1);
 #pragma unroll
             for (int g = 0; g < N2B; ++g) {
                 if (more1) {
 #pragma unroll
                     for (int t = g * LA; t < (g + 1) * LA && t < NL; ++t) {
-                        if (t < 8 && (t & 1) == 0) wfA[t / 2] = FRAG_W(nb, 0, t / 2);
-                        else afA[t < 8 ? t / 2 : t - 4] = FRAG_A(nb, 0, t < 8 ? t / 2 : t - 4);
+                        if (t < 8 && (t & 1) == 0) wfA[t / 2] = FRAG_W(nwb, 0, t / 2);
+                        else afA[t < 8 ? t / 2 : t - 4] = FRAG_A(nab, 0, t < 8 ? t / 2 : t - 4);
                     }
                 }
 #pragma unroll
                 for (int j = 0; j < 4; ++j) acc[HA + g][j] = IBL_MFMA(wfB[j], afB[HA + g], acc[HA + g][j], 0, 0, 0);
-                if (more2) GEMM_SLOT(g, kt + 2);
+                if (SA && HA + g + 1 < MI) afB[HA + g + 1] *= fa;
+                if (more2) GEMM_SLOT(g, kb2, r2);
                 __builtin_amdgcn_sched_barrier(0);
             }
+            kb = kb1;
+            r = r1;
         }
     } else {
     static_assert(NS == 2, "the vmcnt(0) that closes a step leaves no later stage in flight");
@@ -581,7 +605,7 @@
 #endif
 }
 
-template <int EPI, int ACT, bool T256>
+template <int EPI, int ACT, bool T256, int TERMS>
 static int launch_gemm_cfg(const u16* A, int64_t lda, const u16* W, int64_t ldw, int M, int N, int K, const GemmEpi& epi, hipStream_t s) {
     constexpr int BM = T256 ? 256 : 128, BN = BM;
     const int nwg = (N / BN) * ((M + BM - 1) / BM);
@@ -591,7 +615,7 @@
     IBL_HIP_CHECK(hipGetDevice(&dev));
     const unsigned long long bit = 1ull << (dev & 63);
     if (!(attr_set.load(std::memory_order_acquire) & bit)) {
-        IBL_HIP_CHECK(hipFuncSetAttribute(reinterpret_cast<const void*>(&ibl_gemm_f16_tn<EPI, ACT, T256>),
+        IBL_HIP_CHECK(hipFuncSetAttribute(reinterpret_cast<const void*>(&ibl_gemm_f16_tn<EPI, ACT, T256, TERMS>),
                                           hipFuncAttributeMaxDynamicSharedMemorySize, (int)lds));
         attr_set.fetch_or(bit, std::memory_order_release);
     }
@@ -608,7 +632,7 @@
     }
     void* tok;
     ibl_prof_begin(IBL_PROF_GEMM, 2.0 * (double)M * (double)N * (double)(epi.algo_k < 0 ? 0 : (epi.algo_k ? epi.algo_k : K)), s, &tok);
-    hipLaunchKernelGGL((ibl_gemm_f16_tn<EPI, ACT, T256>), dim3(grid), dim3(T256 ? 512 : 256), lds, s, A, lda, W, ldw, M, N, K, epi);
+    hipLaunchKernelGGL((ibl_gemm_f16_tn<EPI, ACT, T256, TERMS>), dim3(grid), dim3(T256 ? 512 : 256), lds, s, A, lda, W, ldw, M, N, K, epi);
     ibl_prof_end(tok, s);
     IBL_LAUNCH_CHECK();
     return IBL_OK;
@@ -620,21 +644,31 @@
     return v == 1;
 }
 
+constexpr bool kx_epilogue(int epi) { return epi != EPI_PATCH_F32 && epi != EPI_RESID_PRE_F32; }
+
 template <int EPI, int ACT>
 static int launch_gemm(const u16* A, int64_t lda, const u16* W, int64_t ldw, int M, int N, int K, const GemmEpi& epi,
-                       hipStream_t s) {
+                       hipStream_t s, int terms) {
     if (M <= 0) return IBL_OK;
     if (N % 128 != 0 || K % GBK != 0)
         return ibl_set_error(IBL_ERR_ARG, "gemm: N (%d) must be a multiple of 128 and K (%d) of 64", N, K);
-    if (N % 256 == 0 && M >= 4096) return launch_gemm_cfg<EPI, ACT, true>(A, lda, W, ldw, M, N, K, epi, s);
-    return launch_gemm_cfg<EPI, ACT, false>(A, lda, W, ldw, M, N, K, epi, s);
-}
-
-int gemm_launch(int epi, int act, const u16* A, int64_t lda, const u16* W, int64_t ldw, int M, int N, int K, const GemmEpi& e, hipStream_t s) {
+    if (terms < 1 || terms > 3 || K % (terms * GBK) != 0)
+        return ibl_set_error(IBL_ERR_ARG, "gemm: %d terms (1, 2 or 3) need K (%d) to be that many blocks of a multiple of 64", terms, K);
+    if (N % 256 == 0 && M >= 4096) {
+        if constexpr (kx_epilogue(EPI)) {
+            if (terms == 2) return launch_gemm_cfg<EPI, ACT, true, 2>(A, lda, W, ldw, M, N, K, epi, s);
+        }
+        return launch_gemm_cfg<EPI, ACT, true, 1>(A, lda, W, ldw, M, N, K, epi, s);
+    }
+    return launch_gemm_cfg<EPI, ACT, false, 1>(A, lda, W, ldw, M, N, K, epi, s);
+}
+
+int gemm_launch(int epi, int act, const u16* A, int64_t lda, const u16* W, int64_t ldw, int M, int N, int K, const GemmEpi& e, hipStream_t s,
+                int terms) {
     if (epi < EPI_BIAS_H16 || epi > EPI_BIAS_GELU_H16KX3) return ibl_set_error(IBL_ERR_ARG, "%s: unknown epilogue %d", "gemm", epi);
     switch (act * 8 + epi) {
 #define GEMM_ROW(EPI, ACT) \
-    case (ACT) * 8 + (EPI): return launch_gemm<EPI, ACT>(A, lda, W, ldw, M, N, K, e, s)
+    case (ACT) * 8 + (EPI): return launch_gemm<EPI, ACT>(A, lda, W, ldw, M, N, K, e, s, terms)
         GEMM_ROW(EPI_BIAS_H16, IBL_ACT_GELU_ERF);
         GEMM_ROW(EPI_BIAS_GELU_H16, IBL_ACT_GELU_ERF);
         GEMM_ROW(EPI_RESID_F32, IBL_ACT_GELU_ERF);
@@ -665,7 +699,7 @@
     return a >= 1.17549435e-38f && a <= 3.0e38f && frexpf(a, &e) == 0.5f;
 }
 
-static int linear_f16_run(const ibl_linear_desc* d, int act, int act_max, void* stream, const char* fn);
+static int linear_f16_run(const ibl_linear_desc* d, int act, int act_max, void* stream, const char* fn, int kx_terms = 1);
 
 extern "C" int ibl_linear_f16_ex(const ibl_linear_desc* d, void* stream) {
     if (!d) return ibl_set_error(IBL_ERR_ARG, "ibl_linear_f16_ex: null descriptor");
@@ -683,7 +717,15 @@
     return linear_f16_run(d, activation, IBL_ACT_GELU_TANH, stream, "ibl_linear_f16_act");
 }
 
-static int linear_f16_run(const ibl_linear_desc* d, int act, int act_max, void* stream, const char* fn) {
+extern "C" int ibl_test_linear_f16_terms(const ibl_linear_desc* d, int activation, int terms, void* stream) {
+    if (!d) return ibl_set_error(IBL_ERR_ARG, "ibl_test_linear_f16_terms: null descriptor");
+    if (d->activation != 0 || activation < IBL_ACT_GELU_ERF || activation > IBL_ACT_GELU_TANH)
+        return ibl_set_error(IBL_ERR_ARG, "ibl_test_linear_f16_terms: activation %d (0, 1 or 2; the descriptor's field 0)", activation);
+    if (d->rows == 0) return IBL_OK;
+    return linear_f16_run(d, activation, IBL_ACT_GELU_TANH, stream, "ibl_test_linear_f16_terms", terms);
+}
+
+static int linear_f16_run(const ibl_linear_desc* d, int act, int act_max, void* stream, const char* fn, int kx_terms) {
     if (!d->x || !d->W || !d->out) return ibl_set_error(IBL_ERR_ARG, "%s: null operand", fn);
     if (d->rows < 0 || d->rows > 0x7fffffff) return ibl_set_error(IBL_ERR_ARG, "%s: rows out of range", fn);
     const int n_out = d->n_out, n_in = d->n_in, epi = d->epilogue;
@@ -719,7 +761,7 @@
         e.accumulate = d->accumulate;
     }
     return gemm_launch(epi, act, reinterpret_cast<const u16*>(d->x), d->ldx, reinterpret_cast<const u16*>(d->W), d->ldw, (int)d->rows, n_out, n_in,
-                       e, reinterpret_cast<hipStream_t>(stream));
+                       e, reinterpret_cast<hipStream_t>(stream), kx_terms);
 }
 
 extern "C" int ibl_linear_f16(const void* x, int64_t ldx, const void* W, int64_t ldw, const float* bias, const float* scale,
diff --git a/instance-based-loc_amd/csrc/vit_kernels.h b/instance-based-loc_amd/csrc/vit_kernels.h
--- a/instance-based-loc_amd/csrc/vit_kernels.h
+++ b/instance-based-loc_amd/csrc/vit_kernels.h
@@ -47,7 +47,7 @@
 #define VIT_INTERNAL __attribute__((visibility("hidden")))
 
 VIT_INTERNAL int gemm_launch(int epi, int act, const u16* A, int64_t lda, const u16* W, int64_t ldw, int M, int N, int K, const GemmEpi& e,
-                             hipStream_t s);
+                             hipStream_t s, int terms = 1);
 VIT_INTERNAL bool gemm_resid_pre();
 VIT_INTERNAL int launch_layernorm(const float* x, int64_t ld_x, int64_t n_rows, int dim, const float* g, const float* b, float eps, void* out,
                                   int64_t ld_out, int terms, hipStream_t s);
diff --git a/instance-based-loc_amd/csrc/vit_ragged.hip b/instance-based-loc_amd/csrc/vit_ragged.hip
--- a/instance-based-loc_amd/csrc/vit_ragged.hip
+++ b/instance-based-loc_amd/csrc/vit_ragged.hip
@@ -104,7 +104,7 @@
     e.bias = bias; e.scale = ls; e.out = out; e.ldo = D; e.alpha = 1.0f; e.algo_k = K;
     const int64_t kx = (int64_t)terms * K;
     int st = gemm_launch((ls || !gemm_resid_pre()) ? IBL_LINEAR_RESID_F32 : IBL_LINEAR_RESID_PRE_F32, IBL_ACT_GELU_ERF, a, lda,
-                         reinterpret_cast<const u16*>(terms > 1 ? w_x : w), kx, rows, D, (int)kx, e, c.s);
+                         reinterpret_cast<const u16*>(terms > 1 ? w_x : w), kx, rows, D, (int)kx, e, c.s, terms);
     if (st) return st;
     if (!cls_only && terms == 1 && w_lo) {
         e.bias = nullptr; e.scale = ls_lo; e.algo_k = -1; e.alpha = 1.0f / IBL_VIT_SPLIT_SCALE;
@@ -124,7 +124,7 @@
         GemmEpi e{};
         e.bias = L->b_qkv; e.out = c.qkv; e.ldo = 3 * D; e.algo_k = D;
         st = gemm_launch(IBL_LINEAR_F16, IBL_ACT_GELU_ERF, c.xn, (int64_t)t.qkv * D, reinterpret_cast<const u16*>(t.qkv > 1 ? L->w_qkv_x : L->w_qkv),
-                         (int64_t)t.qkv * D, (int)c.Rn, 3 * D, t.qkv * D, e, c.s);
+                         (int64_t)t.qkv * D, (int)c.Rn, 3 * D, t.qkv * D, e, c.s, t.qkv);
         if (st) return st;
         st = run_attention_ragged(c.qkv, c.att, c.seq_off, c.batch, c.max_tokens, D, H, 0, c.s, t.o);
         if (st) return st;
@@ -161,7 +161,7 @@
     const int epi = t.fc2 == 3 ? IBL_LINEAR_GELU_F16_X3 : (t.fc2 == 2 ? IBL_LINEAR_GELU_F16_X2 : IBL_LINEAR_GELU_F16);
     const int act = (d->flags & IBL_VIT_QUICK_GELU) ? IBL_ACT_QUICK_GELU : ((d->flags & IBL_VIT_TANH_GELU) ? IBL_ACT_GELU_TANH : IBL_ACT_GELU_ERF);
     st = gemm_launch(epi, act, mlp_in, (int64_t)t.fc1 * D, reinterpret_cast<const u16*>(t.fc1 > 1 ? L->w_fc1_x : L->w_fc1), (int64_t)t.fc1 * D, mlp_rows,
-                     d->mlp_dim, t.fc1 * D, e, c.s);
+                     d->mlp_dim, t.fc1 * D, e, c.s, t.fc1);
     if (st) return st;
     return resid_gemm(c, t.cls_only, t.cls_only ? c.cx : c.x, c.hid, (int64_t)t.fc2 * d->mlp_dim, mlp_rows, t.fc2, d->mlp_dim, L->w_fc2,
                       L->w_fc2_x, L->w_fc2_lo, L->b_fc2, L->ls2, L->ls2_lo);
```

After: 792.5 query-frames/s. -4.8%, worse.
